# Ruslan361/iterative_solvers

Measured on AMD Instinct MI355X. Metric: cg_iters_per_sec, higher is better.
Workload: dtype f64; 1 GPU; 4096x4096 L-shaped Dirichlet Poisson fp64, matrix-free CG, fixed 2641 iterations; n=4096, unknowns=12574721, rule=rel2

## Files before the change

include/mi355cg.h:

```cpp
#ifndef MI355CG_H
#define MI355CG_H

#include <stddef.h>

#ifdef __cplusplus
extern "C" {
#endif

#define MI355CG_OK            0
#define MI355CG_ERR_INVALID   1
#define MI355CG_ERR_HIP       2
#define MI355CG_ERR_STATE     3

#define MI355CG_F64           0
#define MI355CG_F32_MIXED     1

#define MI355CG_RULE_MSG_MAXNORM  0
#define MI355CG_RULE_REL_2NORM    1

#define MI355CG_STOP_ITERATIONS   0
#define MI355CG_STOP_PRECISION    1
#define MI355CG_STOP_RESIDUAL     2
#define MI355CG_STOP_EXACT_ERROR  3
#define MI355CG_STOP_INTERRUPTED  4
// ... 48 lines not shown
int  mi355cg_set_rhs(mi355cg_handle h, const double *b);
int  mi355cg_setup_on_device(mi355cg_handle h);

int  mi355cg_apply(mi355cg_handle h, const double *x, double *y);
int  mi355cg_apply_device(mi355cg_handle h, const double *x_dev, double *y_dev);

void mi355cg_default_params(mi355cg_params *p, int rule);
int  mi355cg_solve(mi355cg_handle h, const mi355cg_params *params,
                   mi355cg_iter_cb cb, void *user, const volatile int *stop_flag,
                   mi355cg_results *out);
int  mi355cg_get_solution(mi355cg_handle h, double *x);
int  mi355cg_get_recursive_residual(mi355cg_handle h, double *r);
int  mi355cg_get_true_residual(mi355cg_handle h, double *ax_minus_b);

#define MI355CG_PRECOND_NONE    0
#define MI355CG_PRECOND_MG      1
#define MI355CG_PRECOND_MG_ANY  2
int  mi355cg_set_preconditioner(mi355cg_handle h, int kind);
int  mi355cg_apply_preconditioner(mi355cg_handle h, const double *r, double *z);
int  mi355cg_mg_levels(int n, int *levels, int *coarsest_n);
int  mi355cg_mg_hierarchy(int kind, int n, int max_levels, int *levels, int *level_n);

#define MI355CG_CYCLE_F64 0
#define MI355CG_CYCLE_F32 1
int  mi355cg_set_preconditioner_ex(mi355cg_handle h, int kind, int cycle);
int  mi355cg_preconditioner_info(mi355cg_handle h, int *kind, int *cycle, int *levels);

#define MI355CG_SMOOTHER_JACOBI    0
#define MI355CG_SMOOTHER_LINE_X    1
#define MI355CG_SMOOTHER_LINE_Y    2
#define MI355CG_SMOOTHER_LINE_AUTO 3
int  mi355cg_set_smoother(mi355cg_handle h, int smoother);
int  mi355cg_get_smoother(mi355cg_handle h, int *smoother, int *direction);

#define MI355CG_BATCH_MAX 64
int  mi355cg_solve_batch(mi355cg_handle h, const mi355cg_params *params, int nrhs, const double *b, double *x,
                         const volatile int *stop_flag, mi355cg_results *out);
int  mi355cg_solve_batch_device(mi355cg_handle h, const mi355cg_params *params, int nrhs, const double *b_dev, double *x_dev,
                                const volatile int *stop_flag, mi355cg_results *out);
int  mi355cg_batch_release(mi355cg_handle h);

int  mi355cg_set_initial_guess(mi355cg_handle h, const double *x0);
int  mi355cg_set_initial_guess_device(mi355cg_handle h, const double *x0_dev);
int  mi355cg_use_solution_as_initial_guess(mi355cg_handle h);
int  mi355cg_solve_batch_from(mi355cg_handle h, const mi355cg_params *params, int nrhs, const double *b, double *x,
                              const volatile int *stop_flag, mi355cg_results *out);
int  mi355cg_solve_batch_device_from(mi355cg_handle h, const mi355cg_params *params, int nrhs, const double *b_dev, double *x_dev,
                                     const volatile int *stop_flag, mi355cg_results *out);

int  mi355cg_set_shift(mi355cg_handle h, double sigma);
int  mi355cg_get_shift(mi355cg_handle h, double *sigma);
int  mi355cg_time_steps(mi355cg_handle h, const mi355cg_params *params, double tau, double theta, int nsteps,
                        const volatile int *stop_flag, mi355cg_results *out , int *steps_done);
int  mi355cg_get_solution_device(mi355cg_handle h, double *x_dev);

#define MI355CG_EIG_BLOCK_MAX 16
#define MI355CG_EIG_CONVERGED   0
#define MI355CG_EIG_ITERATIONS  1
#define MI355CG_EIG_INTERRUPTED 2
#define MI355CG_EIG_BREAKDOWN   3
typedef struct mi355cg_eig_results {
    int iterations;
    int converged;
    int stop_reason;
    int p_drops;
    double solve_seconds;
} mi355cg_eig_results;
int  mi355cg_eigs(mi355cg_handle h, int nev, int block, double tol, int max_iterations, double *x, double *lambda, double *resid,
                  const volatile int *stop_flag, mi355cg_eig_results *out);
int  mi355cg_eigs_device(mi355cg_handle h, int nev, int block, double tol, int max_iterations, double *x_dev, double *lambda,
                         double *resid, const volatile int *stop_flag, mi355cg_eig_results *out);
int  mi355cg_eigs_release(mi355cg_handle h);
int  mi355cg_block_gram(mi355cg_handle h, int na, const double *a, int nb, const double *b, double *c);
int  mi355cg_block_gram_indexed(mi355cg_handle h, int na, const double *a, int nia, const int *ia, int nb, const double *b,
                                int nib, const int *ib, double *c);
int  mi355cg_block_combine(mi355cg_handle h, int k, const double *s, int m, const double *coef, double *y);
int  mi355cg_rayleigh_ritz(int k, const double *g, const double *hmat, double *theta, double *coef);

int  mi355cg_set_profiling(mi355cg_handle h, int enable);
int  mi355cg_get_kernel_time(mi355cg_handle h, int kernel, double *avg_ms, long long *launches);
int  mi355cg_get_layout(mi355cg_handle h, long long *padded_len, int *pitch_bottom, int *pitch_upper,
                        int *grid_stencil, int *grid_update, int *rows_per_item);
int  mi355cg_get_xfold(mi355cg_handle h, int *depth, int *extra_buffers);

#define MI355CG_SOLVE_LAUNCHES 0
#define MI355CG_SOLVE_ONCHIP   1
int  mi355cg_set_solve_mode(mi355cg_handle h, int mode);
int  mi355cg_get_solve_mode(mi355cg_handle h, int *mode, long long *onchip_launches_last_solve);
int  mi355cg_onchip_plan(int n, int *threads, int *lds_bytes, int *elems_per_thread);

#define MI355CG_MANY_MAX 65536
int  mi355cg_solve_many(mi355cg_handle h, const mi355cg_params *params, int nsys, const double *b, double *x, const double *sigma,
                        const volatile int *stop_flag, mi355cg_results *out);
int  mi355cg_solve_many_from(mi355cg_handle h, const mi355cg_params *params, int nsys, const double *b, double *x, const double *sigma,
                             const volatile int *stop_flag, mi355cg_results *out);
int  mi355cg_solve_many_device(mi355cg_handle h, const mi355cg_params *params, int nsys, const double *b_dev, double *x_dev,
                               const double *sigma_dev, const volatile int *stop_flag, mi355cg_results *out);
int  mi355cg_solve_many_device_from(mi355cg_handle h, const mi355cg_params *params, int nsys, const double *b_dev, double *x_dev,
                                    const double *sigma_dev, const volatile int *stop_flag, mi355cg_results *out);
int  mi355cg_solve_many_info(mi355cg_handle h, int nsys, int *lds_bytes_per_workgroup, int *workgroups_per_cu, long long *workspace_bytes);

int  mi355cg_slab_rows(int n, int world, int rank, int *y_lo, int *y_hi);
int  mi355cg_create_part(int n, int m, double a, double b, double c, double d, int dtype, int device,
                         int y_lo, int y_hi, int x_lo, int x_hi, mi355cg_handle *out);
int  mi355cg_checksum(mi355cg_handle h, int which, double *out2);
int  mi355cg_create_slab(int n, int m, double a, double b, double c, double d, int dtype, int device,
                         int y_lo, int y_hi, mi355cg_handle *out);
int  mi355cg_owned_range(mi355cg_handle h, long long *packed_begin, long long *packed_len, int *y_lo, int *y_hi);
int  mi355cg_dist_begin(mi355cg_handle h, const mi355cg_params *params, void *stream);
int  mi355cg_dist_reduce(mi355cg_handle h, int which , int with_rows, void *stream);
int  mi355cg_dist_sums_ptr(mi355cg_handle h, int which, void **dev_ptr, int *count );
int  mi355cg_dist_record_layout(mi355cg_handle h, int *header, int *row_slot, int *width);
int  mi355cg_dist_scatter_ghosts(mi355cg_handle h, int vector ,
                                 const double *gathered_records, int nranks, int rank, void *stream);
int  mi355cg_dist_stencil(mi355cg_handle h, const double *gathered_update_sums, int nranks, int estride,
                          int rows , void *stream);
int  mi355cg_dist_flip(mi355cg_handle h);
int  mi355cg_dist_update(mi355cg_handle h, const double *gathered_stencil_sums, int nranks, int estride,
                         int rows , void *stream);
int  mi355cg_dist_update_reads_ghosts(mi355cg_handle h);
int  mi355cg_dist_check(mi355cg_handle h, const double *gathered_update_sums, int nranks, int estride, void *stream);
int  mi355cg_dist_summary(mi355cg_handle h, mi355cg_results *out, int *done);
int  mi355cg_dist_finish(mi355cg_handle h, void *stream);
int  mi355cg_dist_history(mi355cg_handle h, int iteration, double *precision, double *residual, double *error);
int  mi355cg_dist_halo(mi355cg_handle h, int vector ,
                       void **send_lo, void **recv_lo, long long *n_send_lo,
                       void **send_hi, void **recv_hi, long long *n_send_hi);
int  mi355cg_dist_halo_recv_counts(mi355cg_handle h, long long *n_from_lo, long long *n_from_hi);

#define MI355CG_DECOMP_ROWS 0
#define MI355CG_DECOMP_2D   1
typedef struct mi355cg_team_s *mi355cg_team;
typedef struct mi355cg_halo_msg {
    int id;
    int peer;
    int send;
    int kind;
    int y0, y1, x0, x1;
    long long count;
} mi355cg_halo_msg;
int  mi355cg_decompose(int n, int world, int decomp, int rank, int *y_lo, int *y_hi, int *x_lo, int *x_hi);
int  mi355cg_halo_plan(int n, int world, int decomp, int rank, int max_msgs, int *n_msgs, mi355cg_halo_msg *msgs);
int  mi355cg_debug_plan(int n, int world, int decomp, int rank, int which, int *n_panels, int *panels,
                        int *grid, int *n_items, int *cls);
int  mi355cg_team_create_local(int n, int m, double a, double b, double c, double d, int world,
                               const int *devices, int ndevices, int decomp, mi355cg_team *out);
int  mi355cg_team_unique_id(void *id128);
int  mi355cg_team_create_rccl(int n, int m, double a, double b, double c, double d, int world, int rank, int device,
                              const void *id128, int decomp, mi355cg_team *out);
void mi355cg_team_destroy(mi355cg_team t);
int  mi355cg_team_solve(mi355cg_team t, const mi355cg_params *params, mi355cg_iter_cb cb, void *user,
                        const volatile int *stop_flag, mi355cg_results *out);
int  mi355cg_team_info(mi355cg_team t, int *world, int *nlocal, int *decomp, long long *size);
int  mi355cg_team_describe(mi355cg_team t, char *buf, int len);
int  mi355cg_team_part(mi355cg_team t, int local_index, mi355cg_handle *part, int *rank);
int  mi355cg_team_get_vector(mi355cg_team t, int which, double *global_packed);
int  mi355cg_team_checksum(mi355cg_team t, int which, double *out2);
int  mi355cg_team_set_vector(mi355cg_team t, int which, const double *global_packed);
int  mi355cg_team_set_dtype(mi355cg_team t, int dtype);
int  mi355cg_team_setup_on_device(mi355cg_team t);
int  mi355cg_team_set_profiling(mi355cg_team t, int enable);
int  mi355cg_team_phase_times(mi355cg_team t, double *kernel_ms, double *comm_ms, double *wall_ms);

#ifdef __cplusplus
}
#endif
// ... 2 lines not shown
```

iterative_solvers_amd/_capi.py:

```python
from __future__ import annotations

import ctypes as C
import os

import numpy as np

from . import build as _build

OK, ERR_INVALID, ERR_HIP, ERR_STATE = 0, 1, 2, 3
F64, F32_MIXED = 0, 1
RULE_MSG_MAXNORM, RULE_REL_2NORM = 0, 1
STOP_ITERATIONS, STOP_PRECISION, STOP_RESIDUAL, STOP_EXACT_ERROR, STOP_INTERRUPTED = range(5)

EXPORTS = [
    "mi355cg_create", "mi355cg_create_csr", "mi355cg_set_true_solution", "mi355cg_destroy", "mi355cg_last_error", "mi355cg_version", "mi355cg_size",
    "mi355cg_get_rhs", "mi355cg_get_true_solution", "mi355cg_get_node_coords", "mi355cg_set_rhs",
    "mi355cg_apply", "mi355cg_apply_device", "mi355cg_default_params", "mi355cg_solve",
    "mi355cg_get_solution", "mi355cg_get_recursive_residual", "mi355cg_get_true_residual",
    "mi355cg_set_profiling", "mi355cg_get_kernel_time", "mi355cg_get_layout",
    "mi355cg_slab_rows", "mi355cg_create_slab", "mi355cg_owned_range", "mi355cg_dist_begin",
    "mi355cg_dist_reduce", "mi355cg_dist_sums_ptr", "mi355cg_dist_record_layout", "mi355cg_dist_scatter_ghosts", "mi355cg_dist_stencil", "mi355cg_dist_flip",
    "mi355cg_dist_update", "mi355cg_dist_update_reads_ghosts", "mi355cg_dist_check", "mi355cg_dist_summary", "mi355cg_dist_finish", "mi355cg_dist_history",
    "mi355cg_dist_halo", "mi355cg_dist_halo_recv_counts",
    "mi355cg_create_part", "mi355cg_checksum", "mi355cg_decompose", "mi355cg_halo_plan",
    "mi355cg_team_create_local", "mi355cg_team_unique_id", "mi355cg_team_create_rccl", "mi355cg_team_destroy",
    "mi355cg_team_solve", "mi355cg_team_info", "mi355cg_team_part", "mi355cg_team_get_vector", "mi355cg_team_set_vector", "mi355cg_team_checksum",
    "mi355cg_team_set_profiling", "mi355cg_team_phase_times", "mi355cg_team_describe", "mi355cg_setup_on_device", "mi355cg_team_setup_on_device", "mi355cg_debug_plan",
    "mi355cg_team_set_dtype", "mi355cg_set_preconditioner", "mi355cg_apply_preconditioner", "mi355cg_mg_levels",
    "mi355cg_mg_hierarchy", "mi355cg_set_preconditioner_ex", "mi355cg_preconditioner_info",
    "mi355cg_solve_batch", "mi355cg_solve_batch_device", "mi355cg_batch_release", "mi355cg_get_xfold",
    "mi355cg_set_initial_guess", "mi355cg_set_initial_guess_device", "mi355cg_use_solution_as_initial_guess",
    "mi355cg_solve_batch_from", "mi355cg_solve_batch_device_from",
    "mi355cg_set_shift", "mi355cg_get_shift", "mi355cg_time_steps", "mi355cg_get_solution_device",
    "mi355cg_eigs", "mi355cg_eigs_device", "mi355cg_eigs_release", "mi355cg_block_gram", "mi355cg_block_gram_indexed",
    "mi355cg_block_combine", "mi355cg_rayleigh_ritz",
    "mi355cg_set_smoother", "mi355cg_get_smoother",
    "mi355cg_set_solve_mode", "mi355cg_get_solve_mode", "mi355cg_onchip_plan",
    "mi355cg_solve_many", "mi355cg_solve_many_from", "mi355cg_solve_many_device", "mi355cg_solve_many_device_from", "mi355cg_solve_many_info",
]
DECOMP_ROWS, DECOMP_2D = 0, 1
PRECOND_NONE, PRECOND_MG, PRECOND_MG_ANY = 0, 1, 2
CYCLE_F64, CYCLE_F32 = 0, 1
SOLVE_LAUNCHES, SOLVE_ONCHIP = 0, 1
SMOOTHER_JACOBI, SMOOTHER_LINE_X, SMOOTHER_LINE_Y, SMOOTHER_LINE_AUTO = 0, 1, 2, 3
BATCH_MAX = 64
MANY_MAX = 65536
EIG_BLOCK_MAX = 16
EIG_BASIS_MAX = 48
EIG_CONVERGED, EIG_ITERATIONS, EIG_INTERRUPTED, EIG_BREAKDOWN = range(4)


class Params(C.Structure):
    _fields_ = [("rule", C.c_int), ("max_iterations", C.c_int),
                ("eps_precision", C.c_double), ("eps_residual", C.c_double),
                ("eps_exact_error", C.c_double), ("eps_rel", C.c_double),
                ("use_true_solution", C.c_int), ("callback_every", C.c_int),
                ("diagnostics", C.c_int), ("sync_every", C.c_int), ("fixed_iterations", C.c_int),
                ("inner_eps", C.c_double)]


class Results(C.Structure):
    _fields_ = [("iterations", C.c_int), ("converged", C.c_int), ("stop_reason", C.c_int),
                ("final_residual_norm", C.c_double), ("final_precision", C.c_double),
                ("final_error_norm", C.c_double), ("r_norm2", C.c_double),
                ("initial_r_norm2", C.c_double), ("solve_seconds", C.c_double),
                ("refine_true_rel", C.c_double), ("refine_outer", C.c_int), ("loop_seconds", C.c_double)]


class EigResults(C.Structure):
    _fields_ = [("iterations", C.c_int), ("converged", C.c_int), ("stop_reason", C.c_int), ("p_drops", C.c_int),
                ("solve_seconds", C.c_double)]


class HaloMsg(C.Structure):
    _fields_ = [("id", C.c_int), ("peer", C.c_int), ("send", C.c_int), ("kind", C.c_int),
                ("y0", C.c_int), ("y1", C.c_int), ("x0", C.c_int), ("x1", C.c_int), ("count", C.c_longlong)]


ITER_CB = C.CFUNCTYPE(None, C.c_void_p, C.c_int, C.c_double, C.c_double, C.c_double)
_DP = np.ctypeslib.ndpointer(dtype=np.float64, flags="C_CONTIGUOUS")

_lib = None


class Mi355cgError(RuntimeError):
    def __init__(self, code: int, text: str):
        super().__init__(f"mi355cg error {code}: {text}")
        self.code = code


def lib_path() -> str:
    return _build.LIB_PATH


def load():
    global _lib
    if _lib is not None:
        return _lib
    path = os.environ.get("MI355CG_LIB") or _build.LIB_PATH
    if path == _build.LIB_PATH and _build.needs_build():
        try:
            _build.build()
        except Exception as e:
            if not os.path.exists(path):
                raise RuntimeError(f"libmi355cg.so is missing and could not be built: {e}") from e
    try:
        import torch
    except ImportError:
        pass
    L = C.CDLL(path)
    H = C.c_void_p
    L.mi355cg_create.argtypes = [C.c_int, C.c_int] + [C.c_double] * 4 + [C.c_int, C.c_int, C.POINTER(H)]
    _IPn = np.ctypeslib.ndpointer(dtype=np.int32, flags="C_CONTIGUOUS")
# ... 18 lines not shown
    L.mi355cg_get_kernel_time.argtypes = [H, C.c_int, C.POINTER(C.c_double), C.POINTER(C.c_longlong)]
    L.mi355cg_get_layout.argtypes = [H, C.POINTER(C.c_longlong)] + [C.POINTER(C.c_int)] * 5
    LLP, IP, VPP = C.POINTER(C.c_longlong), C.POINTER(C.c_int), C.POINTER(C.c_void_p)
    L.mi355cg_slab_rows.argtypes = [C.c_int, C.c_int, C.c_int, IP, IP]
    L.mi355cg_create_slab.argtypes = [C.c_int, C.c_int] + [C.c_double] * 4 + [C.c_int] * 4 + [C.POINTER(H)]
    L.mi355cg_owned_range.argtypes = [H, LLP, LLP, IP, IP]
    L.mi355cg_dist_begin.argtypes = [H, C.POINTER(Params), C.c_void_p]
    L.mi355cg_dist_reduce.argtypes = [H, C.c_int, C.c_int, C.c_void_p]
    L.mi355cg_dist_sums_ptr.argtypes = [H, C.c_int, VPP, IP]
    L.mi355cg_dist_record_layout.argtypes = [H, IP, IP, IP]
    L.mi355cg_dist_scatter_ghosts.argtypes = [H, C.c_int, C.c_void_p, C.c_int, C.c_int, C.c_void_p]
    L.mi355cg_dist_stencil.argtypes = [H, C.c_void_p, C.c_int, C.c_int, C.c_int, C.c_void_p]
    L.mi355cg_dist_flip.argtypes = [H]
    L.mi355cg_dist_update.argtypes = [H, C.c_void_p, C.c_int, C.c_int, C.c_int, C.c_void_p]
    L.mi355cg_dist_update_reads_ghosts.argtypes = [H]
    L.mi355cg_dist_check.argtypes = [H, C.c_void_p, C.c_int, C.c_int, C.c_void_p]
    L.mi355cg_dist_summary.argtypes = [H, C.POINTER(Results), IP]
    L.mi355cg_dist_finish.argtypes = [H, C.c_void_p]
    DBP = C.POINTER(C.c_double)
    L.mi355cg_dist_history.argtypes = [H, C.c_int, DBP, DBP, DBP]
    L.mi355cg_dist_halo.argtypes = [H, C.c_int, VPP, VPP, LLP, VPP, VPP, LLP]
    L.mi355cg_dist_halo_recv_counts.argtypes = [H, LLP, LLP]
    L.mi355cg_create_part.argtypes = [C.c_int, C.c_int] + [C.c_double] * 4 + [C.c_int] * 6 + [C.POINTER(H)]
    L.mi355cg_checksum.argtypes = [H, C.c_int, DBP]
    L.mi355cg_decompose.argtypes = [C.c_int] * 4 + [IP] * 4
    L.mi355cg_halo_plan.argtypes = [C.c_int] * 5 + [IP, C.POINTER(HaloMsg)]
    L.mi355cg_team_create_local.argtypes = [C.c_int, C.c_int] + [C.c_double] * 4 + [C.c_int, IP, C.c_int, C.c_int, C.POINTER(H)]
    L.mi355cg_team_unique_id.argtypes = [C.c_void_p]
    L.mi355cg_team_create_rccl.argtypes = [C.c_int, C.c_int] + [C.c_double] * 4 + [C.c_int, C.c_int, C.c_int, C.c_void_p, C.c_int, C.POINTER(H)]
    L.mi355cg_team_destroy.argtypes = [H]
    L.mi355cg_team_destroy.restype = None
    L.mi355cg_team_solve.argtypes = [H, C.POINTER(Params), ITER_CB, C.c_void_p, C.c_void_p, C.POINTER(Results)]
    L.mi355cg_team_info.argtypes = [H, IP, IP, IP, LLP]
    L.mi355cg_team_part.argtypes = [H, C.c_int, C.POINTER(H), IP]
    L.mi355cg_team_get_vector.argtypes = [H, C.c_int, _DP]
    L.mi355cg_team_set_vector.argtypes = [H, C.c_int, _DP]
    L.mi355cg_team_checksum.argtypes = [H, C.c_int, DBP]
    L.mi355cg_debug_plan.argtypes = [C.c_int] * 5 + [IP, IP, IP, IP, IP]
    L.mi355cg_setup_on_device.argtypes = [H]
    L.mi355cg_team_setup_on_device.argtypes = [H]
    L.mi355cg_team_set_dtype.argtypes = [H, C.c_int]
    L.mi355cg_team_set_profiling.argtypes = [H, C.c_int]
    L.mi355cg_team_phase_times.argtypes = [H, DBP, DBP, DBP]
    L.mi355cg_team_describe.argtypes = [H, C.c_char_p, C.c_int]
    L.mi355cg_set_preconditioner.argtypes = [H, C.c_int]
    L.mi355cg_set_preconditioner_ex.argtypes = [H, C.c_int, C.c_int]
    L.mi355cg_preconditioner_info.argtypes = [H, IP, IP, IP]
    L.mi355cg_apply_preconditioner.argtypes = [H, _DP, _DP]
    L.mi355cg_mg_levels.argtypes = [C.c_int, IP, IP]
    L.mi355cg_mg_hierarchy.argtypes = [C.c_int, C.c_int, C.c_int, IP, IP]
    L.mi355cg_solve_batch.argtypes = [H, C.POINTER(Params), C.c_int, C.c_void_p, C.c_void_p, C.c_void_p, C.POINTER(Results)]
    L.mi355cg_solve_batch_device.argtypes = [H, C.POINTER(Params), C.c_int, C.c_void_p, C.c_void_p, C.c_void_p, C.POINTER(Results)]
    L.mi355cg_batch_release.argtypes = [H]
    L.mi355cg_set_initial_guess.argtypes = [H, C.c_void_p]
    L.mi355cg_set_initial_guess_device.argtypes = [H, C.c_void_p]
    L.mi355cg_use_solution_as_initial_guess.argtypes = [H]
    L.mi355cg_solve_batch_from.argtypes = [H, C.POINTER(Params), C.c_int, C.c_void_p, C.c_void_p, C.c_void_p, C.POINTER(Results)]
    L.mi355cg_solve_batch_device_from.argtypes = [H, C.POINTER(Params), C.c_int, C.c_void_p, C.c_void_p, C.c_void_p, C.POINTER(Results)]
    L.mi355cg_set_shift.argtypes = [H, C.c_double]
    L.mi355cg_get_shift.argtypes = [H, DBP]
    L.mi355cg_time_steps.argtypes = [H, C.POINTER(Params), C.c_double, C.c_double, C.c_int, C.c_void_p, C.POINTER(Results), IP]
    L.mi355cg_get_solution_device.argtypes = [H, C.c_void_p]
    if hasattr(L, "mi355cg_eigs"):
        for fn in (L.mi355cg_eigs, L.mi355cg_eigs_device):
            fn.argtypes = [H, C.c_int, C.c_int, C.c_double, C.c_int, C.c_void_p, C.c_void_p, C.c_void_p, C.c_void_p, C.POINTER(EigResults)]
        L.mi355cg_eigs_release.argtypes = [H]
        L.mi355cg_block_gram.argtypes = [H, C.c_int, C.c_void_p, C.c_int, C.c_void_p, C.c_void_p]
        L.mi355cg_block_gram_indexed.argtypes = [H, C.c_int, C.c_void_p, C.c_int, C.c_void_p, C.c_int, C.c_void_p, C.c_int, C.c_void_p, C.c_void_p]
        L.mi355cg_block_combine.argtypes = [H, C.c_int, C.c_void_p, C.c_int, C.c_void_p, C.c_void_p]
        L.mi355cg_rayleigh_ritz.argtypes = [C.c_int, C.c_void_p, C.c_void_p, C.c_void_p, C.c_void_p]
    if hasattr(L, "mi355cg_set_smoother"):
        L.mi355cg_set_smoother.argtypes = [H, C.c_int]
        L.mi355cg_get_smoother.argtypes = [H, IP, IP]
    if hasattr(L, "mi355cg_set_solve_mode"):
        L.mi355cg_set_solve_mode.argtypes = [H, C.c_int]
        L.mi355cg_get_solve_mode.argtypes = [H, IP, LLP]
        L.mi355cg_onchip_plan.argtypes = [C.c_int, IP, IP, IP]
    if hasattr(L, "mi355cg_solve_many"):
        for fn in (L.mi355cg_solve_many, L.mi355cg_solve_many_from, L.mi355cg_solve_many_device, L.mi355cg_solve_many_device_from):
            fn.argtypes = [H, C.POINTER(Params), C.c_int, C.c_void_p, C.c_void_p, C.c_void_p, C.c_void_p, C.POINTER(Results)]
        L.mi355cg_solve_many_info.argtypes = [H, C.c_int, IP, IP, LLP]
    if hasattr(L, "mi355cg_get_xfold"):
        L.mi355cg_get_xfold.argtypes = [H, IP, IP]
    _lib = L
    return L


def check(rc: int):
    if rc != OK:
        raise Mi355cgError(rc, load().mi355cg_last_error().decode("utf-8", "replace"))
```

iterative_solvers_amd/csrc/cg_kernels.h:

```cpp
#pragma once
#include <hip/hip_runtime.h>
#include <cfloat>
#include <cmath>
#include "solve_loop.h"
#include "item_table.h"

namespace mi355cg {

#ifdef MI355CG_WAVE_TIMING
constexpr int kWtWaves = 16384, kWtStamps = 6;
__device__ unsigned long long g_wave_dbg[2][kWtStamps * kWtWaves];
#define MI355CG_WT_BEGIN unsigned long long wt_[kWtStamps]; for (int i_ = 0; i_ < kWtStamps; ++i_) wt_[i_] = 0; wt_[0] = wall_clock64();
#define MI355CG_WT_STAMP(I) wt_[I] = wall_clock64();
#define MI355CG_WT_MID wt_[kWtStamps - 2] = wall_clock64();
#define MI355CG_WT_END(K) do { if ((threadIdx.x & 63) == 0) { const int w_ = blockIdx.x * 4 + threadIdx.x / 64; \
    if (w_ < kWtWaves) { wt_[kWtStamps - 1] = wall_clock64(); for (int i_ = 0; i_ < kWtStamps; ++i_) g_wave_dbg[K][kWtStamps * w_ + i_] = wt_[i_]; } } } while (0)
#else
#define MI355CG_WT_BEGIN
#define MI355CG_WT_STAMP(I)
#define MI355CG_WT_MID
#define MI355CG_WT_END(K)
#endif

struct StateLite { double alpha, rr, rr_prev, rz, r0norm; int it, done, first, stop; };
// ... 765 lines not shown
    const T alpha = (T)alpha_d;

    dd s_rr = dd_zero(), s_d2 = dd_zero(), s_e2 = dd_zero();
    double s_rmax = 0, s_dmax = 0, s_emax = 0;
    const long long stride = (long long)gridDim.x * kBlock;
    vec_t* __restrict__ X = reinterpret_cast<vec_t*>(a.x);
    vec_t* __restrict__ R = reinterpret_cast<vec_t*>(a.r);
    const vec_t* __restrict__ Pp = reinterpret_cast<const vec_t*>(a.p);
    const vec_t* __restrict__ Q = reinterpret_cast<const vec_t*>(a.ap);
    const vec_t* __restrict__ Uu = reinterpret_cast<const vec_t*>(a.u);

    auto elem = [&](long long i, const vec_t& x0, const vec_t& pv, const vec_t& r0, const vec_t& qv, const vec_t& uv) {
        vec_t xn, rn;
#pragma unroll
        for (int j = 0; j < VEC; ++j) {
            xn[j] = x0[j] + alpha * pv[j];
            rn[j] = r0[j] - alpha * qv[j];
            const double rd = (double)rn[j];
            dd_acc_prod(s_rr, rd, rd);
            s_rmax = fmax(s_rmax, fabs(rd));
            const double dx = (double)(xn[j] - x0[j]);
            s_dmax = fmax(s_dmax, fabs(dx));
            dd_acc_prod(s_d2, dx, dx);
            if (HAS_U) {
                const double ee = (double)(xn[j] - uv[j]);
                s_emax = fmax(s_emax, fabs(ee));
                dd_acc_prod(s_e2, ee, ee);
            }
        }
        X[i] = xn; R[i] = rn;
    };
    long long i = a.begin + (long long)blockIdx.x * kBlock + threadIdx.x;
    const long long end = a.begin + a.nvec;
    for (; i + stride < end; i += 2 * stride) {
        const long long j0 = i, j1 = i + stride;
        const vec_t xa = X[j0], pa = Pp[j0], ra = R[j0], qa = Q[j0];
        const vec_t xb = X[j1], pb = Pp[j1], rb = R[j1], qb = Q[j1];
        vec_t ua{}, ub{}; if (HAS_U) { ua = Uu[j0]; ub = Uu[j1]; }
        elem(j0, xa, pa, ra, qa, ua);
        elem(j1, xb, pb, rb, qb, ub);
    }
    if (i < end) {
        const vec_t x0 = X[i], pv = Pp[i], r0 = R[i], qv = Q[i];
        vec_t uv{}; if (HAS_U) uv = Uu[i];
        elem(i, x0, pv, r0, qv, uv);
    }

    const dd t_rr = block_reduce_dd(s_rr, lds);
    const double t_rmax = block_reduce<true>(s_rmax, lds);
    const double t_dmax = block_reduce<true>(s_dmax, lds);
    const dd t_d2 = block_reduce_dd(s_d2, lds);
    double t_emax = 0; dd t_e2 = dd_zero();
    if (HAS_U) { t_emax = block_reduce<true>(s_emax, lds); t_e2 = block_reduce_dd(s_e2, lds); }
    if (threadIdx.x == 0) {
        const int b = blockIdx.x, st = a.strideB;
        a.partB[FB_RR * st + b] = t_rr.hi; a.partB[(FB_RR + FB_LO) * st + b] = t_rr.lo;
        a.partB[FB_D2 * st + b] = t_d2.hi; a.partB[(FB_D2 + FB_LO) * st + b] = t_d2.lo;
        a.partB[FB_E2 * st + b] = t_e2.hi; a.partB[(FB_E2 + FB_LO) * st + b] = t_e2.lo;
        a.partB[FB_RMAX * st + b] = t_rmax; a.partB[FB_DMAX * st + b] = t_dmax; a.partB[FB_EMAX * st + b] = t_emax;
        if (blockIdx.x == 0) {
            CgState* o = a.s_out;
            if (a.init == 1) {
                *o = CgState{};
                o->first = 1;
            } else {
                copy_state(a.s_out, a.s_in);
                if (a.init == 2) {
                    if (s.done) o->rr = s.rr_prev;
                    o->done = 0; o->reason = 0; o->converged = 0; o->alpha = 0.0; o->r0norm = a.r0norm_resume;
                    for (int i = 0; i < kRing; ++i) o->alpha_hist[i] = 0.0;
                } else { o->it = s.it + 1; o->first = 0; o->alpha = alpha_d; o->rz = rz; o->alpha_hist[(s.it + 1) & (kRing - 1)] = alpha_d; }
            }
        }
    }
}

template <typename T>
struct FreshArgs {
    long long begin, nvec;
    const T* b; T* x; T* r; T* p0; const T* u;
    double* partB; int strideB;
    CgState* s_out;
};
template <typename T, int VEC, bool HAS_U>
__global__ __launch_bounds__(kBlock) void k_init_fresh(const FreshArgs<T> a) {
    typedef typename VecOf<T, VEC>::type vec_t;
    __shared__ double lds[2 * kWaves];
    dd s_rr = dd_zero(), s_e2 = dd_zero();
    double s_rmax = 0, s_emax = 0;
    const long long stride = (long long)gridDim.x * kBlock;
    const vec_t* __restrict__ B = reinterpret_cast<const vec_t*>(a.b);
    const vec_t* __restrict__ Uu = reinterpret_cast<const vec_t*>(a.u);
    vec_t* __restrict__ X = reinterpret_cast<vec_t*>(a.x);
    vec_t* __restrict__ R = reinterpret_cast<vec_t*>(a.r);
    vec_t* __restrict__ P = reinterpret_cast<vec_t*>(a.p0);
    vec_t zero;
#pragma unroll
    for (int j = 0; j < VEC; ++j) zero[j] = (T)0;
    const long long end = a.begin + a.nvec;
    for (long long i = a.begin + (long long)blockIdx.x * kBlock + threadIdx.x; i < end; i += stride) {
        const vec_t bv = B[i];
        vec_t uv; if (HAS_U) uv = Uu[i];
#pragma unroll
        for (int j = 0; j < VEC; ++j) {
            const double rd = (double)bv[j];
            dd_acc_prod(s_rr, rd, rd);
            s_rmax = fmax(s_rmax, fabs(rd));
            if (HAS_U) {
                const double ee = (double)((T)0 - uv[j]);
                s_emax = fmax(s_emax, fabs(ee));
                dd_acc_prod(s_e2, ee, ee);
            }
        }
        X[i] = zero; R[i] = bv; P[i] = zero;
    }
    const dd t_rr = block_reduce_dd(s_rr, lds);
    const double t_rmax = block_reduce<true>(s_rmax, lds);
    double t_emax = 0; dd t_e2 = dd_zero();
    if (HAS_U) { t_emax = block_reduce<true>(s_emax, lds); t_e2 = block_reduce_dd(s_e2, lds); }
    if (threadIdx.x == 0) {
        const int b = blockIdx.x, st = a.strideB;
        a.partB[FB_RR * st + b] = t_rr.hi; a.partB[(FB_RR + FB_LO) * st + b] = t_rr.lo;
        a.partB[FB_D2 * st + b] = 0.0; a.partB[(FB_D2 + FB_LO) * st + b] = 0.0;
        a.partB[FB_E2 * st + b] = t_e2.hi; a.partB[(FB_E2 + FB_LO) * st + b] = t_e2.lo;
        a.partB[FB_RMAX * st + b] = t_rmax; a.partB[FB_DMAX * st + b] = 0.0; a.partB[FB_EMAX * st + b] = t_emax;
        if (blockIdx.x == 0) { *a.s_out = CgState{}; a.s_out->first = 1; }
    }
}

template <typename T>
struct GuessArgs {
    long long begin, nvec;
    const T* b; const T* ax; const T* x; T* r; T* p0; const T* u;
    double* partB; int strideB;
    double* partG; int strideG;
    CgState* s_out;
};
template <typename T, int VEC, bool HAS_U>
__global__ __launch_bounds__(kBlock) void k_init_guess(const GuessArgs<T> a) {
    typedef typename VecOf<T, VEC>::type vec_t;
    __shared__ double lds[2 * kWaves];
    dd s_rr = dd_zero(), s_bb = dd_zero(), s_e2 = dd_zero();
    double s_rmax = 0, s_emax = 0;
    const long long stride = (long long)gridDim.x * kBlock;
    const vec_t* __restrict__ B = reinterpret_cast<const vec_t*>(a.b);
    const vec_t* __restrict__ AX = reinterpret_cast<const vec_t*>(a.ax);
    const vec_t* __restrict__ X = reinterpret_cast<const vec_t*>(a.x);
    const vec_t* __restrict__ Uu = reinterpret_cast<const vec_t*>(a.u);
    vec_t* __restrict__ R = reinterpret_cast<vec_t*>(a.r);
    vec_t* __restrict__ P = reinterpret_cast<vec_t*>(a.p0);
    vec_t zero;
#pragma unroll
    for (int j = 0; j < VEC; ++j) zero[j] = (T)0;
    const long long end = a.begin + a.nvec;
    for (long long i = a.begin + (long long)blockIdx.x * kBlock + threadIdx.x; i < end; i += stride) {
        const vec_t bv = B[i], av = AX[i];
        vec_t xv, uv; if (HAS_U) { xv = X[i]; uv = Uu[i]; }
        vec_t rv;
#pragma unroll
        for (int j = 0; j < VEC; ++j) {
            rv[j] = bv[j] - av[j];
            const double rd = (double)rv[j], bd = (double)bv[j];
            dd_acc_prod(s_rr, rd, rd);
            dd_acc_prod(s_bb, bd, bd);
            s_rmax = fmax(s_rmax, fabs(rd));
            if (HAS_U) {
                const double ee = (double)(xv[j] - uv[j]);
                s_emax = fmax(s_emax, fabs(ee));
                dd_acc_prod(s_e2, ee, ee);
            }
        }
        R[i] = rv; P[i] = zero;
    }
    const dd t_rr = block_reduce_dd(s_rr, lds);
    const double t_rmax = block_reduce<true>(s_rmax, lds);
    double t_emax = 0; dd t_e2 = dd_zero();
    if (HAS_U) { t_emax = block_reduce<true>(s_emax, lds); t_e2 = block_reduce_dd(s_e2, lds); }
    const dd t_bb = block_reduce_dd(s_bb, lds);
    if (threadIdx.x == 0) {
        const int b = blockIdx.x, st = a.strideB;
        a.partB[FB_RR * st + b] = t_rr.hi; a.partB[(FB_RR + FB_LO) * st + b] = t_rr.lo;
        a.partB[FB_D2 * st + b] = 0.0; a.partB[(FB_D2 + FB_LO) * st + b] = 0.0;
        a.partB[FB_E2 * st + b] = t_e2.hi; a.partB[(FB_E2 + FB_LO) * st + b] = t_e2.lo;
        a.partB[FB_RMAX * st + b] = t_rmax; a.partB[FB_DMAX * st + b] = 0.0; a.partB[FB_EMAX * st + b] = t_emax;
        a.partG[b] = t_bb.hi; a.partG[a.strideG + b] = t_bb.lo;
        if (blockIdx.x == 0) { *a.s_out = CgState{}; a.s_out->first = 1; }
    }
}
__global__ __launch_bounds__(kBlock) void k_guess_state(const double* partB, int strideB, const double* partG, int strideG, int n,
                                                        CgState* s, double* norms) {
    __shared__ double lds[2 * kWaves];
    const double rr = dd_value(reduce_parts_dd(partB + FB_RR * strideB, partB + (FB_RR + FB_LO) * strideB, n, 1, lds));
    const double bb = dd_value(reduce_parts_dd(partG, partG + strideG, n, 1, lds));
    if (threadIdx.x == 0) { s->r0norm = sqrt(bb); s->first = 2; norms[0] = sqrt(rr); norms[1] = sqrt(bb); }
}

template <typename T>
struct UpdateStArgs {
    Geom g;
    ItemTab tab;
    const T* p;
    const T* pprev[kRing - 1];
    T* r; T* x; const T* u;
    const double* partA; int nA, strideA, esA;
    RecSrc src;
    double* partB; int strideB, slotB;
    const CgState* s_in; CgState* s_out;
    int rule;
    int reverse;
    const int* stop_req;
    FlagSpec fl;
    QueueSpec dq;
    double* fold_alpha;
    int fold_mask;
};

template <typename T, int VEC, int XM, bool HAS_U, int DEPTH, bool DESC, bool TEAM, bool QUEUE>
__global__ __launch_bounds__(kBlock) void k_update_st(const UpdateStArgs<T> a) {
    static_assert(DEPTH >= 1 && DEPTH <= 3, "see k_stencil");
    typedef typename VecOf<T, VEC>::type vec_t;
    __shared__ double lds[2 * kWaves];
    const Geom& g = a.g;
    const int lane = threadIdx.x & (kWave - 1);
    const int wave = __builtin_amdgcn_readfirstlane(threadIdx.x / kWave);
    MI355CG_WT_BEGIN
    const StartRec rec = start_rec(a.reverse ? a.tab.start_rev : a.tab.start, wave);
    const ItemSeq seq = rec.seq;
    constexpr bool FULL = XM == 1;
    constexpr int NP = XM >= 2 ? XM - 1 : 0;
    struct Raw { vec_t p, r, x, u, pp[NP > 0 ? NP : 1]; T pe; };

    StateLite s{};
    PreParts pre_lean{0.0, 0.0, 0.0, 0.0}, pre_rz_lean{0.0, 0.0, 0.0, 0.0};
    if (!TEAM) {
        s = load_state_lite(a.s_in);
        const rsrc_t rs_part = make_rsrc(a.partA);
        const int fa = a.strideA * (int)sizeof(double);
        pre_lean = prefetch_parts_buf(rs_part, FA_PAP * fa, FA_LO * fa, a.nA, a.esA);
        if (FULL) pre_rz_lean = prefetch_parts_buf(rs_part, FA_RZ * fa, FA_LO * fa, a.nA, a.esA);
    }

    int f_item = seq.first;
    bool f_have = f_item < seq.end;
    ItemAddr F{};
    int f_idx = 0, f_so = 0, f_y = 0;
    rsrc_t rs_p = make_rsrc(a.p), rs_r = rs_p, rs_x = rs_p, rs_u = rs_p;
    rsrc_t rs_pp[NP > 0 ? NP : 1] = {rs_p};
    const int dq_nsub = min(kQueueSubs, (int)(gridDim.x / kXcds)), dq_sub = (int)(blockIdx.x / kXcds) % dq_nsub;
    int* const dq = (QUEUE && a.dq.mine) ? a.dq.mine + ((int)(blockIdx.x % kXcds) * kQueueSubs + dq_sub) * kQueuePitch : nullptr;
    if (QUEUE && a.dq.other && blockIdx.x == 0 && threadIdx.x < kXcds * kQueueSubs) a.dq.other[threadIdx.x * kQueuePitch] = 0;
    int dq_ticket = 0;
    auto enter = [&](const ItemUni& u) {
        if (QUEUE && dq) dq_ticket = queue_take(dq, lane);
        F = item_addr<T, VEC, DESC>(g, u, lane);
        rs_p = make_rsrc(a.p + F.base_el);
        rs_r = make_rsrc(a.r + F.base_el);
        rs_x = make_rsrc(XM != 0 ? a.x + F.base_el : a.p + F.base_el);
#pragma unroll
        for (int i = 0; i < NP; ++i) rs_pp[i] = make_rsrc(a.pprev[i] + F.base_el);
        rs_u = make_rsrc((FULL && HAS_U) ? a.u + F.base_el : a.p + F.base_el);
        f_idx = -1; f_so = F.so_first; f_y = DESC ? F.ystart + 1 : F.ystart - 1;
    };
    auto fetch = [&](bool may_switch = true) -> Raw {
        if (may_switch && f_have && f_idx > F.nrows) {
            f_item = (QUEUE && dq) ? seq.begin + seq.step + __builtin_amdgcn_readfirstlane(dq_ticket) * dq_nsub + dq_sub : f_item + seq.step;
            f_have = f_item < seq.end;
            if (f_have) enter(item_uniform<DESC>(g, decode_item(a.tab, a.reverse ? seq.end - 1 - (f_item - seq.begin) : f_item), (int)sizeof(T)));
        }
        const bool own = f_have && f_idx >= 0 && f_idx < F.nrows;
        int vo = own ? F.vo_own : (f_idx < 0 ? F.vo_first : F.vo_last);
        if (!f_have) vo = kOob;
        const int vown = own ? F.vo_own : kOob;
        Raw w;
        w.p = buf_load<vec_t>(rs_p, vo, f_so);
        w.r = buf_load<vec_t>(rs_r, vown, f_so);
        if (XM != 0) w.x = buf_load<vec_t>(rs_x, vown, f_so);
#pragma unroll
        for (int i = 0; i < NP; ++i) w.pp[i] = buf_load<vec_t>(rs_pp[i], vown, f_so);
        if (FULL && HAS_U) w.u = buf_load<vec_t>(rs_u, vown, f_so);
        w.pe = buf_load<T>(rs_p, own ? F.ve_own : kOob, f_so);
        if (DESC) { f_so -= row_step<T>(g, f_y - 1); --f_y; } else { f_so += row_step<T>(g, f_y); ++f_y; }
        ++f_idx;
        return w;
    };

    bool c_have = f_have;
    ItemAddr C{};
    int c_idx = -1, c_so = 0, c_y = 0;
    bool in_j[VEC];
#pragma unroll
    for (int j = 0; j < VEC; ++j) in_j[j] = false;
    rsrc_t rs_ro = rs_p, rs_xo = rs_p;
    auto promote = [&]() {
        C = F;
        rs_ro = make_rsrc(a.r + C.base_el);
        rs_xo = make_rsrc(XM != 0 ? a.x + C.base_el : a.p + C.base_el);
        c_idx = -1; c_so = C.so_c0; c_y = C.ystart;
        const int xint0 = C.bot ? g.half + 1 : 1;
#pragma unroll
        for (int j = 0; j < VEC; ++j) in_j[j] = (C.x + j >= xint0) && (C.x + j <= g.N - 1);
    };

    if (f_have) { enter(rec.u); promote(); }
    Raw q[DEPTH];
#pragma unroll
    for (int k = 0; k < DEPTH; ++k) q[k] = fetch(false);
    MI355CG_WT_STAMP(3)
    int stop_word = 0;
    if (blockIdx.x == 0 && a.stop_req) stop_word = scalar_load(a.stop_req);

    double alpha_d, rz = 0.0;
    if (!TEAM) {
        if (s.done) { if (blockIdx.x == 0 && threadIdx.x == 0) copy_state(a.s_out, a.s_in); return; }
        MI355CG_WT_STAMP(1)
        const double pap = dd_value(reduce_parts_dd_pre(pre_lean, a.partA + FA_PAP * a.strideA, a.partA + (FA_PAP + FA_LO) * a.strideA, a.nA, a.esA, lds));
        if (a.rule == 0) {
            rz = FULL ? dd_value(reduce_parts_dd_pre(pre_rz_lean, a.partA + FA_RZ * a.strideA, a.partA + (FA_RZ + FA_LO) * a.strideA, a.nA, a.esA, lds))
                      : dd_value(reduce_parts_dd(a.partA + FA_RZ * a.strideA, a.partA + (FA_RZ + FA_LO) * a.strideA, a.nA, a.esA, lds));
            alpha_d = rz / pap;
        } else {
            alpha_d = s.rr / pap;
        }
        MI355CG_WT_STAMP(2)
    } else if (a.src.mbox) {
        __shared__ double recs[kMaxRecDst * kRecWords];
        const PreParts pre = prefetch_parts(a.partA + FA_PAP * a.strideA, a.partA + (FA_PAP + FA_LO) * a.strideA, a.nA, 1);
        PreParts pre_rz{0, 0, 0, 0};
        if (FULL) pre_rz = prefetch_parts(a.partA + FA_RZ * a.strideA, a.partA + (FA_RZ + FA_LO) * a.strideA, a.nA, 1);
        s = load_state_lite(a.s_in);
        if (s.done) {
            if (threadIdx.x == 0) { store_flagged_zero(a.fl, a.slotB + blockIdx.x, FB_LL_COUNT); if (blockIdx.x == 0) copy_state(a.s_out, a.s_in); }
            return;
        }
        {
            double* R = recs + a.src.me * kRecWords;
            if (threadIdx.x < kRecWords) R[threadIdx.x] = 0.0;
            const dd pap = reduce_parts_dd_pre(pre, a.partA + FA_PAP * a.strideA, a.partA + (FA_PAP + FA_LO) * a.strideA, a.nA, 1, lds);
            dd rzd = dd_zero();
            if (a.rule == 0) rzd = FULL ? reduce_parts_dd_pre(pre_rz, a.partA + FA_RZ * a.strideA, a.partA + (FA_RZ + FA_LO) * a.strideA, a.nA, 1, lds)
// ... 101 lines not shown

    MI355CG_WT_END(1);
    const dd t_rr = block_reduce_dd(s_rr, lds);
    const double t_rmax = block_reduce<true>(s_rmax, lds);
    double t_dmax = 0, t_emax = 0; dd t_d2 = dd_zero(), t_e2 = dd_zero();
    if (FULL) { t_dmax = block_reduce<true>(s_dmax, lds); t_d2 = block_reduce_dd(s_d2, lds); }
    if (FULL && HAS_U) { t_emax = block_reduce<true>(s_emax, lds); t_e2 = block_reduce_dd(s_e2, lds); }
    if (threadIdx.x == 0) {
        const int b = a.slotB + blockIdx.x, st = a.strideB;
        a.partB[FB_RR * st + b] = t_rr.hi; a.partB[(FB_RR + FB_LO) * st + b] = t_rr.lo;
        a.partB[FB_D2 * st + b] = t_d2.hi; a.partB[(FB_D2 + FB_LO) * st + b] = t_d2.lo;
        a.partB[FB_E2 * st + b] = t_e2.hi; a.partB[(FB_E2 + FB_LO) * st + b] = t_e2.lo;
        a.partB[FB_RMAX * st + b] = t_rmax; a.partB[FB_DMAX * st + b] = t_dmax; a.partB[FB_EMAX * st + b] = t_emax;
        if (TEAM && a.fl.part) {
            const double v[FB_LL_COUNT] = {t_rr.hi, t_d2.hi, t_e2.hi, t_rr.lo, t_d2.lo, t_e2.lo, t_rmax, t_dmax, t_emax, (blockIdx.x == 0 && stop_word) ? 1.0 : 0.0};
            store_flagged(a.fl, b, FB_LL_COUNT, v);
        }
        if (blockIdx.x == 0) {
            copy_state(a.s_out, a.s_in);
            CgState* o = a.s_out;
            o->it = s.it + 1; o->first = 0; o->alpha = alpha_d; o->rz = rz; o->alpha_hist[(s.it + 1) & (kRing - 1)] = alpha_d;
            o->stop = stop_word != 0;
            if (a.fold_alpha) a.fold_alpha[(s.it + 1) & a.fold_mask] = alpha_d;
        }
    }
}

struct CheckArgs {
    const double* partB; int nB, strideB, esB;
    RecSrc src;
    const CgState* s_in;
    CgState* summary;
    HistEntry* hist;
    RuleParams rp;
    int want_diag;
};
__global__ __launch_bounds__(kBlock) void k_check(const CheckArgs a) {
    __shared__ double lds[2 * kWaves];
    const StateLite s = load_state_lite(a.s_in);
    if (s.done) { if (threadIdx.x == 0) copy_state(a.summary, a.s_in); return; }
    Decision d;
    if (a.src.mbox) {
        __shared__ double recs[kMaxRecDst * kRecWords];
        own_record_B(recs, a.src.me, a.partB, a.nB, a.strideB, 2, lds);
        if (!gather_records(a.src, recs)) { if (threadIdx.x == 0) fail_transport(a.summary, a.s_in); return; }
        d = decide_from_records(s, a.rp, recs, a.src.world, true, true);
    } else d = reduce_and_decide(s, a.rp, a.partB, a.nB, a.strideB, a.esB, 1, lds);
    if (threadIdx.x == 0) write_state_after_decision(a.summary, a.hist, a.s_in, s, d);
}

template <typename T> struct FlushArgs { const T* p[kRing - 1]; T a[kRing - 1]; int n; };
template <typename T, int VEC>
__global__ __launch_bounds__(kBlock) void k_flush_x(const Geom g, const ItemTab tab, T* x, const FlushArgs<T> f) {
    typedef typename VecOf<T, VEC>::type vec_t;
    const int lane = threadIdx.x & (kWave - 1);
    const int wave = __builtin_amdgcn_readfirstlane(threadIdx.x / kWave);
    for (int item = blockIdx.x * kWaves + wave; item < tab.nitems; item += gridDim.x * kWaves) {
        const Item it = decode_item(tab, item);
        const int x0 = it.strip * (kWave * VEC) + lane * VEC;
        if (x0 < (it.ya <= g.half ? g.cb : 0) || x0 >= g.xlim) continue;
        for (int y = it.ya; y <= it.yb; ++y) {
            const long long off = row_off(g, y) - g.base0 + x0;
            vec_t xn = *reinterpret_cast<const vec_t*>(x + off);
#pragma unroll
            for (int k = 0; k < kRing - 1; ++k) if (k < f.n) {
                const vec_t pv = *reinterpret_cast<const vec_t*>(f.p[k] + off);
#pragma unroll
                for (int j = 0; j < VEC; ++j) xn[j] = xn[j] + f.a[k] * pv[j];
            }
            *reinterpret_cast<vec_t*>(x + off) = xn;
        }
    }
}

constexpr int kFoldMax = 32;
struct FoldTable { const double* p[kFoldMax]; double alpha[kFoldMax]; };
struct FoldArgs {
    long long begin, nvec;
    double* x;
    const FoldTable* tab;
    const CgState* s;
    int mask;
    int flush_it;
};
template <int NS, bool NT>
__device__ inline void fold_block(VecOf<double, 2>::type& xv, const FoldTable* tab, int k0, int mask, long long i) {
    typedef VecOf<double, 2>::type vec_t;
    const vec_t* P[NS]; double al[NS]; vec_t v[NS];
#pragma unroll
    for (int j = 0; j < NS; ++j) {
        const int slot = (k0 + j) & mask;
        P[j] = reinterpret_cast<const vec_t*>(scalar_load(&tab->p[slot]));
        al[j] = scalar_load(&tab->alpha[slot]);
    }
#pragma unroll
    for (int j = 0; j < NS; ++j) v[j] = NT ? __builtin_nontemporal_load(P[j] + i) : P[j][i];
#pragma unroll
    for (int j = 0; j < NS; ++j) { xv[0] = xv[0] + al[j] * v[j][0]; xv[1] = xv[1] + al[j] * v[j][1]; }
}
template <bool NT>
__global__ __launch_bounds__(kBlock) void k_fold_x(const FoldArgs a) {
    typedef VecOf<double, 2>::type vec_t;
    const int it = a.flush_it >= 0 ? a.flush_it : scalar_load(&a.s->it);
    int n = it & a.mask;
    if (a.flush_it < 0) {
        if (scalar_load(&a.s->done) || n != 0 || it == 0) return;
        n = a.mask + 1;
    }
    if (n == 0) return;
    vec_t* __restrict__ X = reinterpret_cast<vec_t*>(a.x);
    const long long stride = (long long)gridDim.x * kBlock, end = a.begin + a.nvec;
    for (long long i = a.begin + (long long)blockIdx.x * kBlock + threadIdx.x; i < end; i += stride) {
        vec_t xv = X[i];
        int k = it - n + 1;
        for (; k + 8 <= it + 1; k += 8) fold_block<8, NT>(xv, a.tab, k, a.mask, i);
        if (k + 4 <= it + 1) { fold_block<4, NT>(xv, a.tab, k, a.mask, i); k += 4; }
        if (k + 2 <= it + 1) { fold_block<2, NT>(xv, a.tab, k, a.mask, i); k += 2; }
        if (k <= it) fold_block<1, NT>(xv, a.tab, k, a.mask, i);
        X[i] = xv;
    }
}

template <typename T, int VEC>
__global__ __launch_bounds__(kBlock) void k_checksum(const Geom g, const ItemTab tab, const T* v, double* part) {
    typedef typename VecOf<T, VEC>::type vec_t;
    __shared__ double lds[2 * kWaves];
    const int lane = threadIdx.x & (kWave - 1);
    const int wave = __builtin_amdgcn_readfirstlane(threadIdx.x / kWave);
    dd s1 = dd_zero(), s2 = dd_zero();
    for (int item = blockIdx.x * kWaves + wave; item < tab.nitems; item += gridDim.x * kWaves) {
        const Item it = decode_item(tab, item);
        const int x0 = it.strip * (kWave * VEC) + lane * VEC;
        if (x0 < (it.ya <= g.half ? g.cb : 0) || x0 >= g.xlim) continue;
        for (int y = it.ya; y <= it.yb; ++y) {
            const vec_t t = *reinterpret_cast<const vec_t*>(v + (row_off(g, y) - g.base0 + x0));
#pragma unroll
            for (int j = 0; j < VEC; ++j) { s1 = dd_add(s1, dd{(double)t[j], 0.0}); dd_acc_prod(s2, (double)t[j], (double)t[j]); }
        }
    }
    const dd t1 = block_reduce_dd(s1, lds), t2 = block_reduce_dd(s2, lds);
    if (threadIdx.x == 0) {
        const int n = gridDim.x, b = blockIdx.x;
        part[b] = t1.hi; part[n + b] = t1.lo; part[2 * n + b] = t2.hi; part[3 * n + b] = t2.lo;
    }
}

template <typename T>
__global__ __launch_bounds__(kBlock) void k_err_maxnorm(long long begin, long long len, const T* x, const T* u, double* part) {
    __shared__ double lds[2 * kWaves];
    const long long stride = (long long)gridDim.x * kBlock;
    double m = 0.0;
    for (long long i = begin + (long long)blockIdx.x * kBlock + threadIdx.x; i < begin + len; i += stride)
        m = fmax(m, fabs((double)(x[i] - u[i])));
    const double t = block_reduce<true>(m, lds);
    if (threadIdx.x == 0) part[blockIdx.x] = t;
}

__global__ __launch_bounds__(kBlock) void k_residual_to_f32(long long total, long long own_begin, long long own_len,
                                                           const double* b, const double* ax, float* rf, double* part) {
    __shared__ double lds[2 * kWaves];
    const long long stride = (long long)gridDim.x * kBlock;
    double s = 0.0;
    for (long long i = (long long)blockIdx.x * kBlock + threadIdx.x; i < total; i += stride) {
        const double d = b[i] - ax[i];
        rf[i] = (float)d;
        if (i >= own_begin && i < own_begin + own_len) s += d * d;
    }
    const double t = block_reduce<false>(s, lds);
    if (threadIdx.x == 0) part[blockIdx.x] = t;
}
__global__ __launch_bounds__(kBlock) void k_accumulate_f32(long long begin, long long len, double* x, const float* d) {
    const long long stride = (long long)gridDim.x * kBlock;
    for (long long i = begin + (long long)blockIdx.x * kBlock + threadIdx.x; i < begin + len; i += stride) x[i] += (double)d[i];
}

struct RecordArgs {
    const double* part; int n, stride;
    int nsum, lo_off;
    int max_first, nmax;
    double* rec; int header, row_slot;
    const double* v; long long off_lo, off_hi; int len_lo, len_hi;
};
__global__ __launch_bounds__(kBlock) void k_make_record(const RecordArgs a) {
    __shared__ double lds[2 * kWaves];
    if (blockIdx.x == 0) {
        for (int f = 0; f < a.nsum; ++f) {
            const dd t = reduce_parts_dd(a.part + f * a.stride, a.part + (f + a.lo_off) * a.stride, a.n, 1, lds);
            if (threadIdx.x == 0) { a.rec[f] = t.hi; a.rec[f + a.lo_off] = t.lo; }
        }
        for (int f = a.max_first; f < a.max_first + a.nmax; ++f) {
            const double t = reduce_parts<true>(a.part + f * a.stride, a.n, 1, lds);
            if (threadIdx.x == 0) a.rec[f] = t;
        }
        return;
    }
    if (!a.v) return;
// ... 90 lines not shown
```

iterative_solvers_amd/csrc/mi355cg.hip:

```cpp
#include "../../include/mi355cg.h"
#include "cg_kernels.h"
#include "device_buffer.h"
#include "csr_kernels.h"
#include "grid_setup.h"
#include "mg_kernels.h"
#include "mg_batch_kernels.h"
#include "eig_kernels.h"
#include "mg_line_kernels.h"
#include "mg_kernels_f32.h"
#include "step_kernels.h"
#include "onchip_kernels.h"

#include <algorithm>
#include <cfloat>
#include <chrono>
#include <cstdarg>
#include <cstddef>
#include <cstdint>
#include <cstdio>
#include <cstdlib>
#include <cstring>
#include <memory>
#include <string>
#include <thread>
// ... 110 lines not shown
    Buf<double> mat_h;
    Buf<double> red;
    Buf<double> stage;
};

struct OnchipManyWs {
    int cap = 0;
    Buf<double> vec;
    Buf<double> small;
    Buf<CgState> s, summary;
    Buf<int> done;
    Buf<CgState> summary_h;
    Buf<double> small_h;
    Buf<int> done_h;
    Buf<double> stage;
    long long stage_cap = 0;
};

}

struct mi355cg_ctx {
    int device = 0;
    int dtype = MI355CG_F64;
    hipStream_t stream = nullptr;
    GridParams gp;
    Geom g{};
    int s_lo = 0, s_hi = 0;
    long long storage_len = 0;
    long long pk_begin = 0, pk_len = 0;
    PackGeom pg{};
    Plan whole, interior, edge;
    Plan whole32;
    Buf<ItemDesc> plan_items[4];
    Buf<StartRec> plan_start[4][2];
    int depth = 2;
    bool has_gc = false;
    int nB_own = 0;
    int strideA = 0, strideB = 0;

    Buf<double> x, r, p[kRing], ap, b, u;
    int xsteps = 4;
    Buf<double> scratch[2];
    Buf<float> xf, rf, pf[kRing], apf;
    Buf<double> packed;
    Buf<double> partA, partB, partR;
    Buf<double> sumsA, sumsB;
    int rec_width = 0;
    mi355cg_params dist_prm{};
    bool dist_active = false, is_slab = false;
    Buf<CgState> sA, sB, summary;
    Buf<int> qctr;
    int dyn_rows = 0;
    Buf<int> stop_h;
    int* stop_dev = nullptr;
    Buf<HistEntry> hist;
    Buf<CgState> summary_h;
    Buf<HistEntry> hist_h;
    Buf<double> partR_h;

    std::vector<double> rhs_h, u_h;
    bool host_rhs_valid = true, host_u_valid = true;
    bool have_u_dev = false, solved = false;
    bool guess_pending = false;
    bool x_is_guess = false;
    Buf<double> guess_part;
    Buf<double> guess_norms_h;
    double sigma = 0.0;
    int smoother = MI355CG_SMOOTHER_JACOBI;
    Buf<double> step_b;
    bool is_csr = false;
    long long csr_n = 0, csr_nnz = 0;
    Buf<int> csr_row_map, csr_entries; Buf<double> csr_values;
    int grid_csr = 0, grid_update = 0;
    int cur = 0;
    int nA_dist = 0;
    int xfold = 0;
    double* fold_p[kFoldMax] = {};
    Buf<double> fold_own[kFoldMax];
    int fold_extra = 0;
    Buf<FoldTable> fold_tab;
    int fcur = 0;
    int fold_grid = 0;
    bool fold_nt = true;

    struct ChunkGraph { int m, cur; std::vector<char> flags; hipGraphExec_t exec; };
    std::vector<ChunkGraph> graphs;
    mi355cg_params graph_prm{};
    bool graph_stop = false;
    int use_graph = -1;
    int solve_mode = MI355CG_SOLVE_LAUNCHES;
    long long onchip_launches = 0;

    hipEvent_t ev_loop[2] = {nullptr, nullptr};
    std::unique_ptr<MgHier> mg;
    std::unique_ptr<MgBatchWs> batch;
    std::unique_ptr<EigWs> eig;
    std::unique_ptr<OnchipManyWs> many;
    bool profiling = false;
    EventPool events;
    std::vector<std::pair<hipEvent_t, hipEvent_t>> ev_pairs[2];
    double kernel_ms[2] = {0, 0};
    long long kernel_launches[2] = {0, 0};
};

namespace {

long long phys_start(const Geom& g, int y) { return row_off(g, y) + (y <= g.half ? g.cb : 0); }
long long phys_end(const Geom& g, int y) { return phys_start(g, y) + (y <= g.half ? g.Pb : g.Pu); }
int strips_total(const GridParams& gp, int vec) { return (gp.n - 1) / (kWave * vec) + 1; }
int first_bottom_strip(const GridParams& gp, int vec) { return (gp.half + 1) / (kWave * vec); }

void own_cols(const mi355cg_ctx* c, int y, int* xa, int* xb) {
    const int lo = y <= c->gp.half ? c->gp.half + 1 : 1, hi = c->gp.n;
    *xa = std::max(lo, c->s_lo * kStripCols);
    *xb = std::max(*xa, std::min(hi, c->s_hi * kStripCols));
}

void build_geom(mi355cg_ctx* c, int vec, int y_lo, int y_hi) {
    Geom& g = c->g;
    const GridParams& gp = c->gp;
    g.N = gp.n; g.half = gp.half;
    g.Pu = (int)round_up(g.N + 1, 32);
    g.cb = g.half & ~31;
    g.Pb = g.Pu - g.cb;
    g.xlim = (int)round_up(g.N + 1, vec);
    g.y_lo = y_lo; g.y_hi = y_hi;
    g.base0 = 0;
    g.base0 = phys_start(g, y_lo - 1);
    c->storage_len = phys_end(g, y_hi + 1) - g.base0;
    g.own_begin = phys_start(g, y_lo) - g.base0;
    g.own_len = phys_end(g, y_hi) - phys_start(g, y_lo);
    g.A = gp.A; g.xk = gp.x_k; g.yk = gp.y_k;
    PackGeom& pg = c->pg;
    pg.g = g;
    const int yb0 = y_lo, yb1 = std::min(y_hi, gp.half), yu0 = std::max(y_lo, gp.half + 1), yu1 = y_hi;
    int xa = 0, xb = 0;
    pg.nb_rows = std::max(0, yb1 - yb0 + 1); pg.yb0 = yb0;
    own_cols(c, gp.half, &xa, &xb); pg.xb0 = xa; pg.wb = pg.nb_rows ? xb - xa : 0;
    pg.nu_rows = std::max(0, yu1 - yu0 + 1); pg.yu0 = yu0;
    own_cols(c, gp.half + 1, &xa, &xb); pg.xu0 = xa; pg.wu = pg.nu_rows ? xb - xa : 0;
    pg.pk_len = (long long)pg.nb_rows * pg.wb + (long long)pg.nu_rows * pg.wu;
    c->pk_len = pg.pk_len;
    c->pk_begin = packed_row_begin(gp, y_lo);
}

int region_rects(const GridParams& gp, int vec, int ya, int yb, int sa, int sb, Rect out[2]) {
    const int ns_all = strips_total(gp, vec), s0b = first_bottom_strip(gp, vec);
    int nr = 0;
    sb = std::min(sb, ns_all);
    if (ya <= gp.half && yb >= 1) {
        const int s0 = std::max(sa, s0b);
        if (s0 < sb) out[nr++] = Rect{std::max(ya, 1), std::min(yb, gp.half), s0, sb, (sa > s0b ? 1 : 0) | (sb < ns_all ? 2 : 0)};
    }
    if (yb > gp.half && sa < sb)
        out[nr++] = Rect{std::max(ya, gp.half + 1), std::min(yb, gp.n - 1), sa, sb, (sa > 0 ? 1 : 0) | (sb < ns_all ? 2 : 0)};
    return nr;
}

PlanKnobs env_knobs() {
    PlanKnobs kn;
    kn.target_waves = env_int("MI355CG_WAVES", 2048); kn.max_blocks = env_int("MI355CG_BLOCKS", 512);
    { const char* v = getenv("MI355CG_ITEM_ROWS"); kn.item_rows = (v && *v) ? std::max(1, atoi(v)) : 0; }
    kn.xcd_classes = env_int("MI355CG_XCD_CLASSES", 1);
    return kn;
}
Plan make_plan(const std::vector<Rect>& rects, int max_rows, int fixed_ty = 0, int dyn_rows = 0) { return make_plan(rects, env_knobs(), max_rows, fixed_ty, dyn_rows); }
// ... 46 lines not shown
    c->use_graph = env_int("MI355CG_GRAPH", -1);
    c->nB_own = c->whole.grid;
}

template <typename T>
int upload(const std::vector<T>& src, Buf<T>& dst, const char* what = nullptr) {
    Buf<T> fresh;
    if (int rc = Buf<T>::device(fresh, (long long)src.size(), what)) return rc;
    if (hipMemcpy(fresh, src.data(), sizeof(T) * src.size(), hipMemcpyHostToDevice) != hipSuccess) {
        const hipError_t e = hipGetLastError();
        return what ? fail(MI355CG_ERR_HIP, "%s", what) : fail(MI355CG_ERR_HIP, "upload of %zu bytes failed: %s", sizeof(T) * src.size(), hipGetErrorString(e));
    }
    dst = std::move(fresh);
    return MI355CG_OK;
}

int upload_item_tables(mi355cg_ctx* c) {
    int k = 0;
    for (Plan* pl : {&c->whole, &c->interior, &c->edge, &c->whole32}) {
        const int slot = k++;
        if (pl->wl.nitems == 0 || pl->grid == 0) continue;
        if (int rc = upload(build_item_table(pl->wl), c->plan_items[slot])) return rc;
        pl->d_items = c->plan_items[slot];
        pl->elem = pl == &c->whole32 ? (int)sizeof(float) : (int)sizeof(double);
        for (int rev = 0; rev < 2; ++rev) {
            if (int rc = upload(build_start_table(pl->wl, pl->grid, c->g, pl->elem, rev != 0), c->plan_start[slot][rev])) return rc;
            pl->d_start[rev] = c->plan_start[slot][rev];
        }
    }
    return MI355CG_OK;
}
ItemTab item_tab(const Plan& pl) { return ItemTab{pl.d_items, pl.d_start[0], pl.d_start[1], pl.wl.nitems}; }

int flat_grid(long long n) { return (int)std::max<long long>(1, std::min<long long>(2048, (n + kBlock - 1) / kBlock)); }

struct PartSrc { const double* ptr; int n, fstride, estride; RecSrc rec; };
struct Where { hipStream_t stream; const Plan* plan; int slot; };

Where whole_part(const mi355cg_ctx* c) { return Where{c->stream, &c->whole, 0}; }
PartSrc own_partB(const mi355cg_ctx* c) { return PartSrc{c->partB, c->nB_own, c->strideB, 1}; }
PartSrc own_partA(const mi355cg_ctx* c) { return PartSrc{c->partA, c->whole.grid, c->strideA, 1}; }

template <typename T, int VEC> Geom kernel_geom(const mi355cg_ctx* c) { Geom g = c->g; g.xlim = (int)round_up(c->g.N + 1, VEC); return g; }

template <typename T, int VEC>
void launch_apply(const mi355cg_ctx* c, const T* v, T* out, const Where& w) {
    if (w.plan->wl.nitems == 0) return;
    StencilArgs<T> a{};
    a.g = kernel_geom<T, VEC>(c); a.tab = item_tab(*w.plan);
    a.pin = v; a.ap = out; a.partA = nullptr;
    hipLaunchKernelGGL((k_stencil<T, VEC, false, false, 2, false, false, false, false>), dim3(w.plan->grid), dim3(kBlock), 0, w.stream, a);
}

struct IterCfg { RuleParams rp; int want_diag; bool has_u; bool x2 = false; bool fold = false; };

template <typename T, int VEC>
void launch_iteration_stencil(mi355cg_ctx* c, const IterCfg& cfg, const T* r, const Buf<T> p[kRing], const Where& w, const PartSrc& pb, const FlagSpec* fl = nullptr) {
    if (w.plan->wl.nitems == 0) return;
    StencilArgs<T> a{};
    a.g = kernel_geom<T, VEC>(c); a.tab = item_tab(*w.plan);
    a.r = r; a.pin = p[c->cur]; a.pout = p[(c->cur + 1) % c->xsteps]; a.ap = nullptr;
    a.partB = pb.ptr; a.nB = pb.n; a.strideB = pb.fstride; a.esB = pb.estride; a.src = pb.rec;
    a.partA = c->partA; a.strideA = c->strideA; a.slotA = w.slot;
    a.s_in = c->sB; a.s_out = c->sA; a.hist = c->hist; a.rp = cfg.rp; a.want_diag = cfg.want_diag;
    a.store_ghosts = c->is_slab ? 1 : 0;
    if (fl) a.fl = *fl;
    if (VEC == 2 && c->dyn_rows > 0 && w.plan == &c->whole) a.dq = QueueSpec{c->qctr, c->qctr + kXcds * kQueueSubs * kQueuePitch};
    const dim3 grid(w.plan->grid), block(kBlock);
    const bool msg = cfg.rp.rule == MI355CG_RULE_MSG_MAXNORM, gc = c->has_gc, d3 = c->depth == 3;
    const bool team = pb.rec.mbox != nullptr || (fl && fl->part), queue = a.dq.mine != nullptr;
#define MI355CG_ST(MSG, D, GC) do { if (team) hipLaunchKernelGGL((k_stencil<T, VEC, true, MSG, D, true, GC, true, VEC == 2>), grid, block, 0, w.stream, a); \
                                    else if (VEC == 2 && queue) hipLaunchKernelGGL((k_stencil<T, VEC, true, MSG, D, true, GC, false, VEC == 2>), grid, block, 0, w.stream, a); \
                                    else hipLaunchKernelGGL((k_stencil<T, VEC, true, MSG, D, true, GC, false, false>), grid, block, 0, w.stream, a); } while (0)
    if constexpr (VEC == 2) {
        if (msg) { if (gc) { if (d3) MI355CG_ST(true, 3, true); else MI355CG_ST(true, 2, true); } else { if (d3) MI355CG_ST(true, 3, false); else MI355CG_ST(true, 2, false); } }
        else     { if (gc) { if (d3) MI355CG_ST(false, 3, true); else MI355CG_ST(false, 2, true); } else { if (d3) MI355CG_ST(false, 3, false); else MI355CG_ST(false, 2, false); } }
    } else {
        if (d3) MI355CG_ST(false, 3, false); else MI355CG_ST(false, 2, false);
    }
#undef MI355CG_ST
}

template <typename T, int VEC>
void launch_iteration_update(mi355cg_ctx* c, const IterCfg& cfg, T* x, T* r, const Buf<T> p[kRing], const T* u, const Where& w, const PartSrc& pa, const FlagSpec* fl = nullptr) {
    if (w.plan->wl.nitems == 0) return;
    UpdateStArgs<T> a{};
    a.g = kernel_geom<T, VEC>(c); a.tab = item_tab(*w.plan);
    a.p = p[c->cur]; a.r = r; a.x = x; a.u = u;
    for (int i = 0; i < kRing - 1; ++i) a.pprev[i] = p[(c->cur + 2 * kRing * c->xsteps - 1 - i) % c->xsteps];
    a.partA = pa.ptr; a.nA = pa.n; a.strideA = pa.fstride; a.esA = pa.estride; a.src = pa.rec;
    a.partB = c->partB; a.strideB = c->strideB; a.slotB = w.slot;
    a.s_in = c->sA; a.s_out = c->sB; a.rule = cfg.rp.rule; a.reverse = 1;
    if (fl) a.fl = *fl;
    if (VEC == 2 && c->dyn_rows > 0 && w.plan == &c->whole) a.dq = QueueSpec{c->qctr + kXcds * kQueueSubs * kQueuePitch, c->qctr};
    if (cfg.fold) { a.fold_alpha = reinterpret_cast<double*>(reinterpret_cast<char*>(c->fold_tab.get()) + offsetof(FoldTable, alpha)); a.fold_mask = c->xfold - 1; }
    a.stop_req = w.slot == 0 ? c->stop_dev : nullptr;
    const dim3 grid(w.plan->grid), block(kBlock);
    const bool d3 = c->depth == 3 && !(cfg.x2 && c->cur == 0 && c->xsteps == 8);
    const bool team = pa.rec.mbox != nullptr || (fl && fl->part), queue = a.dq.mine != nullptr;
#define MI355CG_UST_D(XM, HASU, D) do { if (team) hipLaunchKernelGGL((k_update_st<T, VEC, XM, HASU, D, true, true, VEC == 2>), grid, block, 0, w.stream, a); \
                                        else if (VEC == 2 && queue) hipLaunchKernelGGL((k_update_st<T, VEC, XM, HASU, D, true, false, VEC == 2>), grid, block, 0, w.stream, a); \
                                        else hipLaunchKernelGGL((k_update_st<T, VEC, XM, HASU, D, true, false, false>), grid, block, 0, w.stream, a); } while (0)
#define MI355CG_UST(XM, HASU) do { if (d3) MI355CG_UST_D(XM, HASU, 3); else MI355CG_UST_D(XM, HASU, 2); } while (0)
    if (cfg.x2) {
        if (c->cur != 0 || cfg.fold) MI355CG_UST(0, false); else if (c->xsteps == 8) MI355CG_UST(8, false); else if (c->xsteps == 4) MI355CG_UST(4, false); else MI355CG_UST(2, false);
    }
    else if constexpr (VEC == 2) { if (cfg.has_u) MI355CG_UST(1, true); else MI355CG_UST(1, false); }
#undef MI355CG_UST
#undef MI355CG_UST_D
}

template <typename T, int VEC>
void launch_update_flat(mi355cg_ctx* c, const IterCfg& cfg, T* x, T* r, const T* p, const T* ap, const T* u, hipStream_t stream,
                        int grid, double resume_r0norm = -1.0) {
    UpdateArgs<T> a{};
    a.begin = c->g.own_begin / VEC; a.nvec = c->g.own_len / VEC;
    a.x = x; a.r = r; a.p = p; a.ap = ap; a.u = u;
    a.partA = c->partA; a.nA = 0; a.strideA = c->strideA; a.esA = 1;
    a.partB = c->partB; a.strideB = c->strideB;
    a.s_in = c->sA; a.s_out = c->sB; a.rule = cfg.rp.rule; a.init = 1;
    if (resume_r0norm >= 0.0) { a.init = 2; a.r0norm_resume = resume_r0norm; a.s_in = c->sB; }
    if (cfg.has_u) hipLaunchKernelGGL((k_update<T, VEC, true>), dim3(grid), dim3(kBlock), 0, stream, a);
    else hipLaunchKernelGGL((k_update<T, VEC, false>), dim3(grid), dim3(kBlock), 0, stream, a);
}

template <typename T, int VEC>
void launch_flush_x(const mi355cg_ctx* c, const Plan& plan, T* x, const Buf<T> p[kRing], const CgState& fin, hipStream_t stream) {
    const int pending = fin.it % c->xsteps;
    if (plan.wl.nitems == 0 || pending == 0) return;
    FlushArgs<T> f{};
    f.n = pending;
    for (int j = 0; j < pending; ++j) { const int k = fin.it - pending + 1 + j; f.p[j] = p[k % c->xsteps]; f.a[j] = (T)fin.alpha_hist[k & (kRing - 1)]; }
    hipLaunchKernelGGL((k_flush_x<T, VEC>), dim3(std::max(1, std::min(1024, (plan.wl.nitems + kWaves - 1) / kWaves))), dim3(kBlock), 0, stream,
                       kernel_geom<T, VEC>(c), item_tab(plan), x, f);
}

void launch_fold_x(const mi355cg_ctx* c, int flush_it, hipStream_t stream) {
    FoldArgs a{};
    a.begin = c->g.own_begin / 2; a.nvec = c->g.own_len / 2;
    a.x = c->x; a.tab = c->fold_tab; a.s = c->sB; a.mask = c->xfold - 1; a.flush_it = flush_it;
    const long long one_shot = (a.nvec + kBlock - 1) / kBlock;
    const int grid = (int)std::max<long long>(1, c->fold_grid > 0 ? std::min<long long>(c->fold_grid, one_shot) : one_shot);
    if (c->fold_nt) hipLaunchKernelGGL((k_fold_x<true>), dim3(grid), dim3(kBlock), 0, stream, a);
    else hipLaunchKernelGGL((k_fold_x<false>), dim3(grid), dim3(kBlock), 0, stream, a);
}
void free_fold_ring(mi355cg_ctx* c) {
    for (int k = c->xsteps; k < kFoldMax; ++k) { c->fold_own[k].reset(); c->fold_p[k] = nullptr; }
    c->fold_tab.reset();
    c->fold_extra = 0;
}
bool ensure_fold_ring(mi355cg_ctx* c) {
    if (c->xfold == 0) return false;
    if (c->fold_tab) return true;
    const size_t bytes = sizeof(double) * (size_t)c->storage_len;
    bool ok = true;
    for (int k = 0; k < c->xfold && ok; ++k) {
        if (k < c->xsteps) { c->fold_p[k] = c->p[k]; continue; }
        ok = Buf<double>::device(c->fold_own[k], c->storage_len) == MI355CG_OK && hipMemsetAsync(c->fold_own[k], 0, bytes, c->stream) == hipSuccess;
        c->fold_p[k] = c->fold_own[k];
    }
    FoldTable t{};
    for (int k = 0; k < c->xfold; ++k) t.p[k] = c->fold_p[k];
    ok = ok && Buf<FoldTable>::device(c->fold_tab, 1) == MI355CG_OK &&
         hipMemcpyAsync(c->fold_tab, &t, sizeof t, hipMemcpyHostToDevice, c->stream) == hipSuccess && hipStreamSynchronize(c->stream) == hipSuccess;
    if (!ok) {
        (void)hipGetLastError();
        hipStreamSynchronize(c->stream);
        free_fold_ring(c);
        c->xfold = 0;
        return false;
    }
    c->fold_extra = c->xfold - c->xsteps;
    return true;
}

void launch_check(mi355cg_ctx* c, const IterCfg& cfg, hipStream_t stream, const PartSrc& pb) {
    CheckArgs a{};
    a.partB = pb.ptr; a.nB = pb.n; a.strideB = pb.fstride; a.esB = pb.estride; a.src = pb.rec;
    a.s_in = c->sB; a.summary = c->summary; a.hist = c->hist; a.rp = cfg.rp; a.want_diag = cfg.want_diag;
    hipLaunchKernelGGL(k_check, dim3(1), dim3(kBlock), 0, stream, a);
}

IterCfg make_cfg(const mi355cg_params* prm) {
    IterCfg cfg{};
    const bool msg = prm->rule == MI355CG_RULE_MSG_MAXNORM;
    cfg.rp.rule = prm->rule; cfg.rp.max_iterations = prm->max_iterations;
    cfg.rp.eps_precision = prm->eps_precision; cfg.rp.eps_residual = prm->eps_residual;
    cfg.rp.eps_exact_error = prm->eps_exact_error; cfg.rp.eps_rel = prm->eps_rel;
    cfg.rp.fixed_iterations = prm->fixed_iterations;
    const bool diag = !msg && prm->diagnostics;
    cfg.has_u = (msg && prm->use_true_solution) || diag;
    cfg.rp.use_u = cfg.has_u ? 1 : 0;
    cfg.want_diag = diag ? 1 : 0;
    cfg.x2 = !msg && !diag;
    return cfg;
}

template <typename T>
int upload_packed(mi355cg_ctx* c, const double* host_packed, T* storage) {
    if (c->is_csr) {
        HIPCK(hipMemcpyAsync(storage, host_packed, sizeof(double) * c->pk_len, hipMemcpyHostToDevice, c->stream));
        HIPCK(hipStreamSynchronize(c->stream));
        return MI355CG_OK;
    }
    if (c->is_slab) HIPCK(hipDeviceSynchronize());
    if (c->pk_len == 0) return MI355CG_OK;
    HIPCK(hipMemcpyAsync(c->packed, host_packed, sizeof(double) * c->pk_len, hipMemcpyHostToDevice, c->stream));
    hipLaunchKernelGGL((k_unpack<T>), dim3(flat_grid(c->pk_len)), dim3(kBlock), 0, c->stream, c->pg, c->packed, storage);
    HIPCK(hipGetLastError());
    HIPCK(hipStreamSynchronize(c->stream));
    return MI355CG_OK;
}
template <typename T>
int download_packed(mi355cg_ctx* c, const T* storage, double* host_packed) {
    if (c->is_csr) {
        HIPCK(hipMemcpyAsync(host_packed, storage, sizeof(double) * c->pk_len, hipMemcpyDeviceToHost, c->stream));
        HIPCK(hipStreamSynchronize(c->stream));
        return MI355CG_OK;
    }
    if (c->is_slab) HIPCK(hipDeviceSynchronize());
    if (c->pk_len == 0) return MI355CG_OK;
    hipLaunchKernelGGL((k_pack<T>), dim3(flat_grid(c->pk_len)), dim3(kBlock), 0, c->stream, c->pg, storage, c->packed);
    HIPCK(hipGetLastError());
    HIPCK(hipMemcpyAsync(host_packed, c->packed, sizeof(double) * c->pk_len, hipMemcpyDeviceToHost, c->stream));
    HIPCK(hipStreamSynchronize(c->stream));
    return MI355CG_OK;
}

int ensure_host_copies(mi355cg_ctx* c) {
    if (!c->host_rhs_valid) { c->rhs_h.resize(c->pk_len); if (int rc = download_packed<double>(c, c->b, c->rhs_h.data())) return rc; c->host_rhs_valid = true; }
    if (!c->host_u_valid) { c->u_h.resize(c->pk_len); if (int rc = download_packed<double>(c, c->u, c->u_h.data())) return rc; c->host_u_valid = true; }
    return MI355CG_OK;
}
int ensure_f32_vectors(mi355cg_ctx* c) {
    if (c->xsteps > 4) return fail(MI355CG_ERR_INVALID, "MI355CG_XSTEPS=8 is fp64 only");
    if (c->whole32.wl.nitems == 0) return fail(MI355CG_ERR_INVALID, "the fp32 kernels march 256-column strips: a part of a 2-D decomposition (cut on 128 columns) cannot run them; use row slabs");
    if (c->g.own_begin % 4 != 0 || c->g.own_len % 4 != 0) return fail(MI355CG_ERR_STATE, "a part's owned range is not a whole number of float4");
    Buf<float>* fv[] = {&c->xf, &c->apf, &c->pf[0], &c->pf[1], &c->pf[2], &c->pf[3]};
    for (int k = 0; k < 2 + c->xsteps; ++k)
        if (!*fv[k]) if (int rc = Buf<float>::device_zeroed(*fv[k], c->storage_len, "fp32 vector allocation failed")) return rc;
    HIPCK(hipDeviceSynchronize());
    return MI355CG_OK;
}

int ensure_u_on_device(mi355cg_ctx* c) {
    if (c->have_u_dev) return MI355CG_OK;
    if (!c->host_u_valid) return fail(MI355CG_ERR_STATE, "no exact solution on host or device");
    if (int rc = upload_packed<double>(c, c->u_h.data(), c->u)) return rc;
    c->have_u_dev = true;
    return MI355CG_OK;
}
int ensure_scratch(mi355cg_ctx* c) {
    for (auto& s : c->scratch) if (!s) { if (int rc = Buf<double>::device_zeroed(s, c->storage_len)) return rc; }
    HIPCK(hipDeviceSynchronize());
    return MI355CG_OK;
}

int ensure_guess_ws(mi355cg_ctx* c) {
    if (!c->guess_part) if (int rc = Buf<double>::device(c->guess_part, 2 * (long long)c->strideB + 2)) return rc;
    if (!c->guess_norms_h) if (int rc = Buf<double>::pinned(c->guess_norms_h, 2)) return rc;
    return MI355CG_OK;
}

void clear_graphs(mi355cg_ctx* c) {
    for (auto& g : c->graphs) hipGraphExecDestroy(g.exec);
    c->graphs.clear();
}

void prof_begin(mi355cg_ctx* c, hipEvent_t* e0) {
    if (!c->profiling) return;
    *e0 = c->events.get();
    if (*e0) hipEventRecord(*e0, c->stream);
}
void prof_end(mi355cg_ctx* c, int k, hipEvent_t e0) {
    if (!c->profiling || !e0) return;
    hipEvent_t e1 = c->events.get();
    if (!e1) return;
    hipEventRecord(e1, c->stream);
    c->ev_pairs[k].push_back({e0, e1});
}
void prof_collect(mi355cg_ctx* c) {
    for (int k = 0; k < 2; ++k) {
        double tot = 0; long long n = 0;
        for (auto& pr : c->ev_pairs[k]) {
            float ms = 0;
            if (hipEventElapsedTime(&ms, pr.first, pr.second) == hipSuccess) { tot += ms; ++n; }
        }
        c->kernel_ms[k] = n ? tot / n : 0.0;
        c->kernel_launches[k] = n;
        c->ev_pairs[k].clear();
    }
    c->events.reset();
}

int fetch_state(mi355cg_ctx* c, hipStream_t st) {
    HIPCK(hipMemcpyAsync(c->summary_h, c->summary, sizeof(CgState), hipMemcpyDeviceToHost, st));
    HIPCK(hipMemcpyAsync(c->hist_h, c->hist, sizeof(HistEntry) * kHist, hipMemcpyDeviceToHost, st));
    return MI355CG_OK;
}
int wait_stream_forwarding_stop(mi355cg_ctx* c, const volatile int* stop_flag) {
    if (!stop_flag) { HIPCK(hipStreamSynchronize(c->stream)); return MI355CG_OK; }
    for (;;) {
        if (*stop_flag) *c->stop_h = 1;
        const hipError_t q = hipStreamQuery(c->stream);
        if (q == hipSuccess) break;
        if (q != hipErrorNotReady) HIPCK(q);
        std::this_thread::yield();
    }
    return MI355CG_OK;
}
int loop_timer_begin(mi355cg_ctx* c, hipStream_t st) {
    if (!c->ev_loop[0]) { HIPCK(hipEventCreate(&c->ev_loop[0])); HIPCK(hipEventCreate(&c->ev_loop[1])); }
    HIPCK(hipEventRecord(c->ev_loop[0], st));
    return MI355CG_OK;
}
int loop_timer_end(mi355cg_ctx* c, hipStream_t st) { HIPCK(hipEventRecord(c->ev_loop[1], st)); return MI355CG_OK; }
double loop_timer_seconds(const mi355cg_ctx* c) {
    float ms = 0;
    return hipEventElapsedTime(&ms, c->ev_loop[0], c->ev_loop[1]) == hipSuccess ? 1e-3 * ms : 0.0;
}

}

namespace {

CsrView csr_view(const mi355cg_ctx* c) { return CsrView{c->csr_n, c->csr_row_map, c->csr_entries, c->csr_values}; }

void launch_csr_spmv(mi355cg_ctx* c, const double* x, double* y, const double* r, const CgState* s_in, double* partA) {
    SpmvArgs a{};
    a.A = csr_view(c); a.x = x; a.y = y; a.r = r; a.s_in = s_in; a.partA = partA; a.strideA = c->strideA;
    hipLaunchKernelGGL(k_csr_spmv, dim3(c->grid_csr), dim3(kBlock), 0, c->stream, a);
}

int solve_csr(mi355cg_ctx* c, const mi355cg_params* prm, mi355cg_iter_cb cb, void* user,
              const volatile int* stop_flag, mi355cg_results* out) {
    if (prm->diagnostics) return fail(MI355CG_ERR_INVALID, "per-iteration diagnostics are not available on CSR handles");
    const bool msg = prm->rule == MI355CG_RULE_MSG_MAXNORM;
    IterCfg cfg = make_cfg(prm);
    if (cfg.has_u && !c->have_u_dev) { cfg.has_u = false; cfg.rp.use_u = 0; }
    const auto t0 = std::chrono::steady_clock::now();
    const size_t bytes = sizeof(double) * c->storage_len;
    HIPCK(hipMemsetAsync(c->x, 0, bytes, c->stream));
    HIPCK(hipMemsetAsync(c->p[0], 0, bytes, c->stream));
    HIPCK(hipMemsetAsync(c->ap, 0, bytes, c->stream));
    HIPCK(hipMemcpyAsync(c->r, c->b, bytes, hipMemcpyDeviceToDevice, c->stream));
    c->cur = 0;
    const PartSrc pA{c->partA, c->grid_csr, c->strideA, 1};
    auto update = [&](bool init, bool with_u) {
        UpdateArgs<double> a{};
        a.begin = 0; a.nvec = c->csr_n;
        a.x = c->x; a.r = c->r; a.p = c->p[0]; a.ap = c->ap; a.u = c->u;
        a.partA = pA.ptr; a.nA = pA.n; a.strideA = pA.fstride; a.esA = 1;
        a.partB = c->partB; a.strideB = c->strideB;
        a.s_in = c->sA; a.s_out = c->sB; a.rule = cfg.rp.rule; a.init = init ? 1 : 0;
        if (with_u) hipLaunchKernelGGL((k_update<double, 1, true>), dim3(c->grid_update), dim3(kBlock), 0, c->stream, a);
        else hipLaunchKernelGGL((k_update<double, 1, false>), dim3(c->grid_update), dim3(kBlock), 0, c->stream, a);
    };
    update(true, cfg.has_u);
    HIPCK(hipGetLastError());
    auto poll = [&]() -> int {
        launch_check(c, cfg, c->stream, own_partB(c));
        if (int rc = fetch_state(c, c->stream)) return rc;
        HIPCK(hipStreamSynchronize(c->stream));
        return MI355CG_OK;
    };
    if (int rc = poll()) return rc;
    const double initial_rnorm2 = c->summary_h->rnorm2;
    if (msg && cb) cb(user, 0, DBL_MAX, c->summary_h->rmax, cfg.has_u ? c->summary_h->emax : DBL_MAX);
    const int sync_every = default_sync_every(prm, msg);
    int it_done = 0;
    bool first_chunk = (cb != nullptr || stop_flag != nullptr);
    bool interrupted = false;
    while (!c->summary_h->done) {
        if (stop_flag && *stop_flag) { interrupted = true; break; }
        const int m = chunk_len(prm, msg, sync_every, it_done, first_chunk);
        first_chunk = false;
        for (int k = 0; k < m; ++k) {
            XpayArgs xa{};
            xa.n = c->csr_n; xa.r = c->r; xa.p = c->p[0];
            xa.partB = c->partB; xa.nB = c->grid_update; xa.strideB = c->strideB; xa.esB = 1;
// ... 1060 lines not shown
    }
    hipLaunchKernelGGL(k_mgb_unpack, dim3(flat_grid(c->pk_len), n), dim3(kBlock), 0, c->stream, c->pg, vlen, (const double*)T.packed, T.vec);
    HIPCK(hipGetLastError());
    return MI355CG_OK;
}

}

extern "C" {

const char* mi355cg_last_error(void) { return g_err.c_str(); }
const char* mi355cg_version(void) { return "mi355cg 0.2 (gfx950)"; }

static const char* onchip_refusal(const mi355cg_ctx* c) {
    static char buf[160];
    if (c->is_csr) return "the on-chip solve keeps the grid's direction in LDS: a CSR handle has no grid";
    if (c->is_slab) return "the on-chip solve is one workgroup on one GPU: this handle owns one part of a decomposed grid";
    if (c->dtype != MI355CG_F64) return "the on-chip solve is fp64 only: this handle was created with MI355CG_F32_MIXED";
    if (c->mg) return "the on-chip solve runs plain CG: this handle has a preconditioner (mi355cg_set_preconditioner(h, MI355CG_PRECOND_NONE) first)";
    if (!onchip_supported(c->gp.n)) {
        snprintf(buf, sizeof buf, "the on-chip solve takes grids up to N = %d (the direction must fit in one CU's LDS): this handle has N = %d", kOnchipMaxN, c->gp.n);
        return buf;
    }
    return nullptr;
}
static int create_state(mi355cg_ctx* c, const char* what) {
    if (int rc = Buf<double>::device_zeroed(c->partA, (long long)FA_COUNT * c->strideA)) return rc;
    if (int rc = Buf<double>::device_zeroed(c->partB, (long long)FB_COUNT * c->strideB)) return rc;
    if (int rc = Buf<double>::device_zeroed(c->partR, 2048)) return rc;
    for (Buf<CgState>* s : {&c->sA, &c->sB, &c->summary}) if (int rc = Buf<CgState>::device_zeroed(*s, 1, what)) return rc;
    if (int rc = Buf<HistEntry>::device_zeroed(c->hist, kHist, what)) return rc;
    if (int rc = Buf<CgState>::pinned(c->summary_h, 1, what)) return rc;
    if (int rc = Buf<HistEntry>::pinned(c->hist_h, kHist, what)) return rc;
    return Buf<double>::pinned(c->partR_h, 2048, what);
}

static int create_impl(int n, int m, double a, double b, double c_, double d, int dtype, int device,
                       int y_lo, int y_hi, int s_lo, int s_hi, bool part, mi355cg_handle* out) {
    if (!out) return fail(MI355CG_ERR_INVALID, "out is null");
    *out = nullptr;
    if (dtype != MI355CG_F64 && dtype != MI355CG_F32_MIXED) return fail(MI355CG_ERR_INVALID, "unknown dtype %d", dtype);
    GridParams gp;
    if (!grid_params_init(&gp, n, m, a, b, c_, d))
        return fail(MI355CG_ERR_INVALID, "grid %dx%d rejected: the L-shaped index map is only consistent for n == m, even, >= 6", n, m);
    int ndev = 0;
    if (hipGetDeviceCount(&ndev) != hipSuccess || ndev <= 0)
        return fail(MI355CG_ERR_HIP, "no HIP device available (libmi355cg has no CPU fallback)");
    if (device < 0 || device >= ndev) return fail(MI355CG_ERR_INVALID, "device %d out of range (0..%d)", device, ndev - 1);
    HIPCK(hipSetDevice(device));

    const int ns_all = strips_total(gp, 2);
    if (!part) { y_lo = 1; y_hi = gp.n - 1; s_lo = 0; s_hi = ns_all; }
    if (y_lo < 1 || y_hi > gp.n - 1 || y_lo > y_hi)
        return fail(MI355CG_ERR_INVALID, "part rows [%d, %d] outside 1..%d", y_lo, y_hi, gp.n - 1);
    if (s_lo < 0 || s_hi > ns_all || s_lo >= s_hi)
        return fail(MI355CG_ERR_INVALID, "part strips [%d, %d) outside 0..%d", s_lo, s_hi, ns_all);
    if (dtype == MI355CG_F32_MIXED && part) return fail(MI355CG_ERR_INVALID, "F32_MIXED is single-GPU only");
    mi355cg_ctx* c = new mi355cg_ctx();
    c->device = device; c->dtype = dtype; c->gp = gp; c->is_slab = part;
    c->s_lo = s_lo; c->s_hi = s_hi;
    build_geom(c, 2, y_lo, y_hi);
    build_plans(c);
    c->strideA = std::max({c->whole.grid, c->interior.grid + c->edge.grid, c->whole32.grid, 1});
    c->strideB = c->strideA;

    int rc = MI355CG_OK;
    auto cleanup = [&]() { mi355cg_destroy(c); return rc; };
    if (hipStreamCreateWithFlags(&c->stream, hipStreamNonBlocking) != hipSuccess) { rc = fail(MI355CG_ERR_HIP, "hipStreamCreate failed"); return cleanup(); }
    if ((rc = upload_item_tables(c))) return cleanup();
    const long long L = c->storage_len;
    { const int m = env_int("MI355CG_XSTEPS", 4); c->xsteps = m == 2 ? 2 : ((m == 8 && dtype == MI355CG_F64) ? 8 : 4); }
    if (!part && dtype == MI355CG_F64 && !getenv("MI355CG_XSTEPS")) {
        const char* xf = getenv("MI355CG_XFOLD");
        const int want = (xf && *xf) ? atoi(xf) : -1;
        if (want == 16 || want == 32) c->xfold = want;
        else if (want < 0 && c->g.own_len >= (4LL << 20)) {
            size_t mem_free = 0, mem_total = 0;
            if (hipMemGetInfo(&mem_free, &mem_total) == hipSuccess)
                for (int R : {32, 16}) if (c->xfold == 0 && sizeof(double) * (size_t)L * (size_t)R <= mem_total / 4) c->xfold = R;
        }
        c->fold_grid = std::max(0, env_int("MI355CG_XFOLD_GRID", 0));
        c->fold_nt = env_int("MI355CG_XFOLD_NT", 1) != 0;
    }
    Buf<double>* vecs[] = {&c->x, &c->r, &c->p[0], &c->p[1], &c->ap, &c->b, &c->u, &c->p[2], &c->p[3], &c->p[4], &c->p[5], &c->p[6], &c->p[7]};
    for (int k = 0; k < 7 + (c->xsteps - 2); ++k) if ((rc = Buf<double>::device_zeroed(*vecs[k], L))) return cleanup();
    if (dtype == MI355CG_F32_MIXED) {
        Buf<float>* fv[] = {&c->xf, &c->rf, &c->pf[0], &c->pf[1], &c->apf, &c->pf[2], &c->pf[3], &c->pf[4], &c->pf[5], &c->pf[6], &c->pf[7]};
        for (int k = 0; k < 5 + (c->xsteps - 2); ++k) if ((rc = Buf<float>::device_zeroed(*fv[k], L, "fp32 vector allocation failed"))) return cleanup();
    }
    if ((rc = Buf<double>::device_zeroed(c->packed, std::max<long long>(c->pk_len, 1)))) return cleanup();
    if ((rc = create_state(c, "state allocation failed"))) return cleanup();
    c->rec_width = kRecHeader + 2 * c->g.Pu;
    if ((rc = Buf<double>::device_zeroed(c->sumsA, c->rec_width))) return cleanup();
    if ((rc = Buf<double>::device_zeroed(c->sumsB, c->rec_width))) return cleanup();
    if ((rc = Buf<int>::device_zeroed(c->qctr, 2 * kXcds * kQueueSubs * kQueuePitch, "queue counter allocation failed"))) return cleanup();
    if ((rc = Buf<int>::pinned(c->stop_h, 1, "stop word allocation failed"))) return cleanup();
    *c->stop_h = 0;
    if (hipDeviceSynchronize() != hipSuccess) { rc = fail(MI355CG_ERR_HIP, "hipDeviceSynchronize failed"); return cleanup(); }

    if (env_int("MI355CG_DEVICE_SETUP", 0)) {
        c->host_rhs_valid = false; c->host_u_valid = false;
        if ((rc = mi355cg_setup_on_device(c))) return cleanup();
    } else {
        c->rhs_h.resize(c->pk_len); c->u_h.resize(c->pk_len);
        grid_fill_box(gp, c->g.y_lo, c->g.y_hi, s_lo * kStripCols, s_hi == ns_all ? gp.n : s_hi * kStripCols, c->rhs_h.data(), c->u_h.data(), nullptr, nullptr);
        if ((rc = upload_packed<double>(c, c->rhs_h.data(), c->b))) return cleanup();
    }
    if (env_int("MI355CG_ONCHIP", 0) == 1 && !onchip_refusal(c)) c->solve_mode = MI355CG_SOLVE_ONCHIP;
    *out = c;
    return MI355CG_OK;
}

int mi355cg_create(int n, int m, double a, double b, double c_, double d, int dtype, int device, mi355cg_handle* out) {
    return create_impl(n, m, a, b, c_, d, dtype, device, 0, 0, 0, 0, false, out);
}
int mi355cg_create_slab(int n, int m, double a, double b, double c_, double d, int dtype, int device,
                        int y_lo, int y_hi, mi355cg_handle* out) {
    GridParams gp;
    if (!grid_params_init(&gp, n, m, a, b, c_, d)) return fail(MI355CG_ERR_INVALID, "grid %dx%d rejected: the L-shaped index map is only consistent for n == m, even, >= 6", n, m);
    return create_impl(n, m, a, b, c_, d, dtype, device, y_lo, y_hi, 0, strips_total(gp, 2), true, out);
}
int mi355cg_create_part(int n, int m, double a, double b, double c_, double d, int dtype, int device,
                        int y_lo, int y_hi, int x_lo, int x_hi, mi355cg_handle* out) {
    GridParams gp;
    if (!grid_params_init(&gp, n, m, a, b, c_, d)) return fail(MI355CG_ERR_INVALID, "grid %dx%d rejected: the L-shaped index map is only consistent for n == m, even, >= 6", n, m);
    const int ns_all = strips_total(gp, 2);
    if (x_lo % kStripCols != 0 || (x_hi % kStripCols != 0 && x_hi < gp.n))
        return fail(MI355CG_ERR_INVALID, "part columns [%d, %d): x-cuts must be multiples of %d", x_lo, x_hi, kStripCols);
    return create_impl(n, m, a, b, c_, d, dtype, device, y_lo, y_hi, x_lo / kStripCols, x_hi >= gp.n ? ns_all : x_hi / kStripCols, true, out);
}

int mi355cg_create_csr(long long nrows, const int* row_map, const int* entries, const double* values,
                       int device, mi355cg_handle* out) {
    if (!out) return fail(MI355CG_ERR_INVALID, "out is null");
    *out = nullptr;
    if (nrows <= 0 || !row_map || !entries || !values) return fail(MI355CG_ERR_INVALID, "bad CSR arguments");
    if (row_map[0] != 0) return fail(MI355CG_ERR_INVALID, "row_map[0] must be 0");
    const long long nnz = row_map[nrows];
    for (long long i = 0; i < nrows; ++i) if (row_map[i + 1] < row_map[i]) return fail(MI355CG_ERR_INVALID, "row_map is not monotone at row %lld", i);
    for (long long j = 0; j < nnz; ++j) if (entries[j] < 0 || entries[j] >= nrows) return fail(MI355CG_ERR_INVALID, "column index %d out of range at entry %lld", entries[j], j);
    int ndev = 0;
    if (hipGetDeviceCount(&ndev) != hipSuccess || ndev <= 0) return fail(MI355CG_ERR_HIP, "no HIP device available (libmi355cg has no CPU fallback)");
    if (device < 0 || device >= ndev) return fail(MI355CG_ERR_INVALID, "device %d out of range (0..%d)", device, ndev - 1);
    HIPCK(hipSetDevice(device));
    mi355cg_ctx* c = new mi355cg_ctx();
    c->device = device; c->dtype = MI355CG_F64; c->is_csr = true;
    c->csr_n = nrows; c->csr_nnz = nnz;
    c->gp.size = nrows; c->pk_begin = 0; c->pk_len = nrows; c->storage_len = nrows; c->pg.pk_len = nrows;
    c->g.own_begin = 0; c->g.own_len = nrows;
    const long long nblk = (nrows + kBlock - 1) / kBlock;
    c->grid_csr = (int)std::max<long long>(1, std::min<long long>(2048, nblk));
    c->grid_update = (int)std::max<long long>(1, std::min<long long>(512, nblk));
    c->strideA = c->grid_csr; c->strideB = c->grid_update; c->nB_own = c->grid_update;
    int rc = MI355CG_OK;
    auto cleanup = [&]() { mi355cg_destroy(c); return rc; };
    if (hipStreamCreateWithFlags(&c->stream, hipStreamNonBlocking) != hipSuccess) { rc = fail(MI355CG_ERR_HIP, "hipStreamCreate failed"); return cleanup(); }
    for (Buf<double>* v : {&c->x, &c->r, &c->p[0], &c->p[1], &c->ap, &c->b, &c->u}) if ((rc = Buf<double>::device_zeroed(*v, nrows))) return cleanup();
    if ((rc = create_state(c, "allocation failed"))) return cleanup();
    if ((rc = Buf<int>::device(c->csr_row_map, nrows + 1, "allocation failed")) || (rc = Buf<int>::device(c->csr_entries, std::max<long long>(nnz, 1), "allocation failed")) ||
        (rc = Buf<double>::device(c->csr_values, std::max<long long>(nnz, 1), "allocation failed"))) return cleanup();
    if (hipMemcpy(c->csr_row_map, row_map, sizeof(int) * (nrows + 1), hipMemcpyHostToDevice) != hipSuccess ||
        hipMemcpy(c->csr_entries, entries, sizeof(int) * nnz, hipMemcpyHostToDevice) != hipSuccess ||
        hipMemcpy(c->csr_values, values, sizeof(double) * nnz, hipMemcpyHostToDevice) != hipSuccess) {
        rc = fail(MI355CG_ERR_HIP, "CSR upload failed"); return cleanup();
    }
    if (hipDeviceSynchronize() != hipSuccess) { rc = fail(MI355CG_ERR_HIP, "hipDeviceSynchronize failed"); return cleanup(); }
// ... 51 lines not shown
int mi355cg_setup_on_device(mi355cg_handle c) {
    if (!c) return fail(MI355CG_ERR_INVALID, "null handle");
    if (c->is_csr) return fail(MI355CG_ERR_INVALID, "a CSR handle has no grid to set up");
    HIPCK(hipSetDevice(c->device));
    if (c->is_slab) HIPCK(hipDeviceSynchronize());
    SetupArgs s{};
    s.pg = c->pg; s.a = c->gp.a; s.c = c->gp.c; s.x_step = c->gp.x_step; s.y_step = c->gp.y_step; s.xk = c->gp.x_k; s.yk = c->gp.y_k;
    s.n = c->gp.n; s.m = c->gp.m;
    if (c->pk_len > 0) hipLaunchKernelGGL(k_setup, dim3(flat_grid(c->pk_len)), dim3(kBlock), 0, c->stream, s, c->b, c->u);
    HIPCK(hipGetLastError());
    HIPCK(hipStreamSynchronize(c->stream));
    c->have_u_dev = true; c->host_rhs_valid = false; c->host_u_valid = false;
    return MI355CG_OK;
}
int mi355cg_set_rhs(mi355cg_handle c, const double* b) {
    if (!c || !b) return fail(MI355CG_ERR_INVALID, "null argument");
    HIPCK(hipSetDevice(c->device));
    c->host_rhs_valid = true;
    c->rhs_h.resize(c->pk_len);
    std::memcpy(c->rhs_h.data(), b, sizeof(double) * c->pk_len);
    return upload_packed<double>(c, c->rhs_h.data(), c->b);
}

int mi355cg_apply_device(mi355cg_handle c, const double* x_dev, double* y_dev) {
    if (!c || !x_dev || !y_dev) return fail(MI355CG_ERR_INVALID, "null argument");
    if (c->is_slab) return fail(MI355CG_ERR_STATE, "this handle owns one part of a decomposed grid: use the mi355cg_team_* / mi355cg_dist_* entry points");
    HIPCK(hipSetDevice(c->device));
    if (c->is_csr) {
        launch_csr_spmv(c, x_dev, y_dev, nullptr, nullptr, nullptr);
        HIPCK(hipGetLastError());
        HIPCK(hipStreamSynchronize(c->stream));
        return MI355CG_OK;
    }
    if (int rc = ensure_scratch(c)) return rc;
    hipLaunchKernelGGL((k_unpack<double>), dim3(flat_grid(c->pk_len)), dim3(kBlock), 0, c->stream, c->pg, x_dev, c->scratch[0]);
    launch_apply<double, 2>(c, c->scratch[0], c->scratch[1], whole_part(c));
    hipLaunchKernelGGL((k_pack<double>), dim3(flat_grid(c->pk_len)), dim3(kBlock), 0, c->stream, c->pg, c->scratch[1], y_dev);
    HIPCK(hipGetLastError());
    HIPCK(hipStreamSynchronize(c->stream));
    return MI355CG_OK;
}

int mi355cg_apply(mi355cg_handle c, const double* x, double* y) {
    if (!c || !x || !y) return fail(MI355CG_ERR_INVALID, "null argument");
    if (c->is_slab) return fail(MI355CG_ERR_STATE, "this handle owns one part of a decomposed grid: use the mi355cg_team_* / mi355cg_dist_* entry points");
    HIPCK(hipSetDevice(c->device));
    if (int rc = ensure_scratch(c)) return rc;
    if (int rc = upload_packed<double>(c, x, c->scratch[0])) return rc;
    if (c->is_csr) launch_csr_spmv(c, c->scratch[0], c->scratch[1], nullptr, nullptr, nullptr);
    else launch_apply<double, 2>(c, c->scratch[0], c->scratch[1], whole_part(c));
    HIPCK(hipGetLastError());
    return download_packed<double>(c, c->scratch[1], y);
}

void mi355cg_default_params(mi355cg_params* p, int rule) {
    if (!p) return;
    std::memset(p, 0, sizeof *p);
    p->rule = rule;
    p->max_iterations = 10000;
    p->eps_precision = 1e-6; p->eps_residual = 1e-6; p->eps_exact_error = 1e-6;
    p->eps_rel = 1e-6;
    p->use_true_solution = 1;
    p->callback_every = rule == MI355CG_RULE_MSG_MAXNORM ? 100 : 1;
    p->diagnostics = 0;
    p->sync_every = 0;
    p->fixed_iterations = 0;
    p->inner_eps = 0.0;
}

static int launch_init_guess(mi355cg_ctx* c, bool has_u) {
    launch_apply<double, 2>(c, c->x, c->scratch[0], whole_part(c));
    GuessArgs<double> f{};
    f.begin = c->g.own_begin / 2; f.nvec = c->g.own_len / 2;
    f.b = c->b; f.ax = c->scratch[0]; f.x = c->x; f.r = c->r; f.p0 = c->p[0]; f.u = c->u;
    f.partB = c->partB; f.strideB = c->strideB; f.partG = c->guess_part; f.strideG = c->strideB; f.s_out = c->sB;
    if (has_u) hipLaunchKernelGGL((k_init_guess<double, 2, true>), dim3(c->whole.grid), dim3(kBlock), 0, c->stream, f);
    else hipLaunchKernelGGL((k_init_guess<double, 2, false>), dim3(c->whole.grid), dim3(kBlock), 0, c->stream, f);
    double* norms = c->guess_part + 2 * (size_t)c->strideB;
    hipLaunchKernelGGL(k_guess_state, dim3(1), dim3(kBlock), 0, c->stream, (const double*)c->partB, c->strideB, (const double*)c->guess_part, c->strideB,
                       c->whole.grid, c->sB, norms);
    HIPCK(hipMemcpyAsync(c->guess_norms_h, norms, sizeof(double) * 2, hipMemcpyDeviceToHost, c->stream));
    return MI355CG_OK;
}
static void launch_init_fresh(mi355cg_ctx* c, bool has_u) {
    FreshArgs<double> f{};
    f.begin = c->g.own_begin / 2; f.nvec = c->g.own_len / 2;
    f.b = c->b; f.x = c->x; f.r = c->r; f.p0 = c->p[0]; f.u = c->u;
    f.partB = c->partB; f.strideB = c->strideB; f.s_out = c->sB;
    if (has_u) hipLaunchKernelGGL((k_init_fresh<double, 2, true>), dim3(c->whole.grid), dim3(kBlock), 0, c->stream, f);
    else hipLaunchKernelGGL((k_init_fresh<double, 2, false>), dim3(c->whole.grid), dim3(kBlock), 0, c->stream, f);
}

static void launch_onchip_chunk(mi355cg_ctx* c, const IterCfg& cfg, const mi355cg_params* prm, int m) {
    OnchipArgs a{};
    a.g = c->g; a.pl = onchip_plan(c->gp.n);
    a.x = c->x; a.r = c->r; a.u = c->u;
    for (int k = 0; k < c->xsteps; ++k) a.p[k] = c->p[k];
    a.xsteps = c->xsteps;
    a.partB = c->partB; a.nB = c->nB_own; a.strideB = c->strideB;
    a.s = c->sB; a.hist = c->hist; a.rp = cfg.rp;
    a.has_u = cfg.has_u ? 1 : 0; a.u_always = cfg.rp.eps_exact_error > 0 ? 1 : 0; a.every = prm->callback_every;
    a.m = m; a.stop_req = c->stop_dev;
    const dim3 grid(1), block(a.pl.threads);
    const bool msg = cfg.rp.rule == MI355CG_RULE_MSG_MAXNORM;
#define MI355CG_OC(E) do { if (msg) hipLaunchKernelGGL((k_onchip<E, true>), grid, block, 0, c->stream, a); \
                           else hipLaunchKernelGGL((k_onchip<E, false>), grid, block, 0, c->stream, a); } while (0)
    switch (a.pl.elems) {
        case 1: MI355CG_OC(1); break;
        case 2: MI355CG_OC(2); break;
        case 4: MI355CG_OC(4); break;
        case 8: MI355CG_OC(8); break;
        case 16: MI355CG_OC(16); break;
        default: MI355CG_OC(kOnchipMaxElems); break;
    }
#undef MI355CG_OC
    c->nB_own = 1;
    ++c->onchip_launches;
}

int mi355cg_solve(mi355cg_handle c, const mi355cg_params* prm, mi355cg_iter_cb cb, void* user,
                  const volatile int* stop_flag, mi355cg_results* out) {
    if (!c || !prm) return fail(MI355CG_ERR_INVALID, "null argument");
    if (prm->rule != MI355CG_RULE_MSG_MAXNORM && prm->rule != MI355CG_RULE_REL_2NORM) return fail(MI355CG_ERR_INVALID, "unknown rule %d", prm->rule);
    if (c->is_slab) return fail(MI355CG_ERR_STATE, "this handle owns one part of a decomposed grid: use the mi355cg_team_* / mi355cg_dist_* entry points");
    HIPCK(hipSetDevice(c->device));
    const bool warm = c->guess_pending;
    c->guess_pending = false;
    c->onchip_launches = 0;
    if (c->is_csr) return solve_csr(c, prm, cb, user, stop_flag, out);
    if (c->dtype == MI355CG_F32_MIXED) return solve_mixed(c, prm, cb, user, stop_flag, out);
    if (c->mg) return solve_mg(c, prm, cb, user, stop_flag, out, warm);
    const bool msg = prm->rule == MI355CG_RULE_MSG_MAXNORM;
    IterCfg cfg0 = make_cfg(prm);
    const bool onchip = c->solve_mode == MI355CG_SOLVE_ONCHIP && cfg0.want_diag == 0;
    if (onchip) cfg0.x2 = false;
    cfg0.fold = cfg0.x2 && ensure_fold_ring(c);
    const IterCfg cfg = cfg0;
    const bool diag = cfg.want_diag != 0, fold = cfg.fold;
    c->nB_own = c->whole.grid;
    if (cfg.has_u) if (int rc = ensure_u_on_device(c)) return rc;
    if (diag || (warm && !(c->scratch[0] && c->scratch[1]))) if (int rc = ensure_scratch(c)) return rc;
    if (warm) if (int rc = ensure_guess_ws(c)) return rc;

    const auto t0 = std::chrono::steady_clock::now();
    c->events.reset(); c->ev_pairs[0].clear(); c->ev_pairs[1].clear();

    c->cur = 0; c->fcur = 0;
    if (c->qctr && c->dyn_rows > 0) HIPCK(hipMemsetAsync(c->qctr, 0, sizeof(int) * 2 * kXcds * kQueueSubs * kQueuePitch, c->stream));
    if (warm) { if (int rc = launch_init_guess(c, cfg.has_u)) return rc; }
    else launch_init_fresh(c, cfg.has_u);
    HIPCK(hipGetLastError());

    *c->stop_h = 0;
    c->stop_dev = nullptr;
    if (stop_flag) HIPCK(hipHostGetDevicePointer((void**)&c->stop_dev, c->stop_h, 0));
    auto wait_stream = [&]() -> int { return wait_stream_forwarding_stop(c, stop_flag); };
    bool polled = false;
    auto poll = [&]() -> int {
        launch_check(c, cfg, c->stream, own_partB(c));
        if (int rc = fetch_state(c, c->stream)) return rc;
        polled = true;
        return wait_stream();
    };
    *c->summary_h = CgState{};
    if (msg && (cb || warm)) {
        if (int rc = poll()) return rc;
        if (cb) cb(user, 0, DBL_MAX, c->summary_h->rmax, cfg.has_u ? c->summary_h->emax : DBL_MAX);
    }
    if (warm)
        if (const int reason = msg_stop_reason(prm, false, 0.0, c->summary_h->rmax, cfg.has_u, c->summary_h->emax)) {
            c->summary_h->done = 1; c->summary_h->converged = 1; c->summary_h->reason = reason;
        }
    if (int rc = loop_timer_begin(c, c->stream)) return rc;

    const int every = prm->callback_every;
    auto need_u = [&](int it) { return diag || cfg.rp.eps_exact_error > 0 || it == 1 || (every > 0 && it % every == 0); };
    const int sync_every = default_sync_every(prm, msg);
    int it_done = 0;
    bool interrupted = false;
    bool first_chunk = cb != nullptr || stop_flag != nullptr;
    if (std::memcmp(&c->graph_prm, prm, sizeof *prm) != 0 || c->graph_stop != (stop_flag != nullptr)) {
        clear_graphs(c); c->graph_prm = *prm; c->graph_stop = stop_flag != nullptr;
    }
    const bool graph_ok = !c->profiling && !diag &&
                          (c->use_graph == 1 || (c->use_graph < 0 && c->g.own_len < (4LL << 20) && prm->max_iterations >= 4 * sync_every));
    while (!c->summary_h->done) {
        if (stop_flag && *stop_flag) { interrupted = true; break; }
        const int m = chunk_len(prm, msg, sync_every, it_done, first_chunk);
        first_chunk = false;
        auto enqueue_chunk = [&]() -> int {
            for (int k = 0; k < m; ++k) {
                hipEvent_t e0 = nullptr;
                Buf<double> pp[kRing];
                if (fold) { pp[c->cur].borrow(c->fold_p[c->fcur]); pp[(c->cur + 1) % c->xsteps].borrow(c->fold_p[(c->fcur + 1) % c->xfold]); }
                const Buf<double>* ring = fold ? pp : c->p;
                prof_begin(c, &e0);
                launch_iteration_stencil<double, 2>(c, cfg, c->r, ring, whole_part(c), own_partB(c));
                c->cur = (c->cur + 1) % c->xsteps;
                if (fold) c->fcur = (c->fcur + 1) % c->xfold;
                prof_end(c, 0, e0);
                prof_begin(c, &e0);
                IterCfg ucfg = cfg;
                ucfg.has_u = cfg.has_u && need_u(it_done + k + 1);
                launch_iteration_update<double, 2>(c, ucfg, c->x, c->r, ring, c->u, whole_part(c), own_partA(c));
                if (fold && c->fcur == 0) launch_fold_x(c, -1, c->stream);
                prof_end(c, 1, e0);
                if (diag) {
                    launch_apply<double, 2>(c, c->x, c->scratch[0], whole_part(c));
                    hipLaunchKernelGGL((k_resid2<double>), dim3(1024), dim3(kBlock), 0, c->stream, c->g.own_begin, c->g.own_len, c->b, c->scratch[0], c->partR);
                    hipLaunchKernelGGL(k_resid2_hist, dim3(1), dim3(kBlock), 0, c->stream, c->partR, 1024, c->sB, c->hist);
                }
            }
            return MI355CG_OK;
        };
        if (onchip) {
            launch_onchip_chunk(c, cfg, prm, m);
        } else if (graph_ok && m >= 8) {
            std::vector<char> flags(m);
            for (int k = 0; k < m; ++k) flags[k] = cfg.has_u && need_u(it_done + k + 1);
            mi355cg_ctx::ChunkGraph* hit = nullptr;
            const int key = fold ? c->fcur : c->cur;
            for (auto& g : c->graphs) if (g.m == m && g.cur == key && g.flags == flags) hit = &g;
            if (!hit) {
                hipGraph_t graph = nullptr; hipGraphExec_t exec = nullptr;
                const int cur0 = c->cur, fcur0 = c->fcur;
                HIPCK(hipStreamBeginCapture(c->stream, hipStreamCaptureModeThreadLocal));
                const int rc = enqueue_chunk();
                const hipError_t e1 = hipStreamEndCapture(c->stream, &graph);
                c->cur = cur0; c->fcur = fcur0;
                if (rc) return rc;
                HIPCK(e1);
                HIPCK(hipGraphInstantiate(&exec, graph, nullptr, nullptr, 0));
                HIPCK(hipGraphDestroy(graph));
                c->graphs.push_back({m, key, flags, exec});
                hit = &c->graphs.back();
            }
            HIPCK(hipGraphLaunch(hit->exec, c->stream));
            c->cur = (c->cur + m) % c->xsteps;
            if (fold) c->fcur = (c->fcur + m) % c->xfold;
        } else {
            if (int rc = enqueue_chunk()) return rc;
        }
        HIPCK(hipGetLastError());
        if (int rc = poll()) return rc;
        const int it_now = c->summary_h->it;
        replay_callbacks(cb, user, prm, *c->summary_h, c->hist_h, it_done, it_now, cfg.has_u, diag);
        it_done = it_now;
    }
    if (int rc = loop_timer_end(c, c->stream)) return rc;
    CgState fin = *c->summary_h;
    c->stop_dev = nullptr;
    if (fin.done && fin.reason == MI355CG_STOP_INTERRUPTED) interrupted = true;
    c->cur = fin.it % c->xsteps;
    if (cfg.x2) {
        if (fold) { c->fcur = fin.it % c->xfold; if (c->fcur != 0) launch_fold_x(c, fin.it, c->stream); }
        else launch_flush_x<double, 2>(c, c->whole, c->x, c->p, fin, c->stream);
        HIPCK(hipGetLastError());
        HIPCK(hipStreamSynchronize(c->stream));
    }
    if (cfg.has_u && fin.it > 0 && !need_u(fin.it)) {
        hipLaunchKernelGGL((k_err_maxnorm<double>), dim3(1024), dim3(kBlock), 0, c->stream, c->g.own_begin, c->g.own_len, c->x, c->u, c->partR);
        HIPCK(hipGetLastError());
        HIPCK(hipMemcpyAsync(c->partR_h, c->partR, sizeof(double) * 1024, hipMemcpyDeviceToHost, c->stream));
        HIPCK(hipStreamSynchronize(c->stream));
        double m = 0; for (int i = 0; i < 1024; ++i) m = std::max(m, c->partR_h[i]);
        fin.emax = m;
    }
    c->solved = true; c->x_is_guess = false;
    prof_collect(c);
#ifdef MI355CG_WAVE_TIMING
    if (const char* path = getenv("MI355CG_WAVE_TIMING_OUT")) {
        std::vector<unsigned long long> buf(2 * kWtStamps * kWtWaves);
        HIPCK(hipMemcpyFromSymbol(buf.data(), HIP_SYMBOL(g_wave_dbg), buf.size() * sizeof(unsigned long long)));
        if (FILE* f = fopen(path, "wb")) { fwrite(buf.data(), sizeof(unsigned long long), buf.size(), f); fclose(f); }
    }
#endif
    mi355cg_results res = make_results(fin, interrupted, cfg.has_u, warm && polled ? c->guess_norms_h[0] : fin.r0norm);
    res.solve_seconds = std::chrono::duration<double>(std::chrono::steady_clock::now() - t0).count();
    HIPCK(hipEventSynchronize(c->ev_loop[1]));
    res.loop_seconds = loop_timer_seconds(c);
    if (msg && cb) cb(user, res.iterations, res.final_precision, res.final_residual_norm, res.final_error_norm);
    if (out) *out = res;
    return MI355CG_OK;
}

int mi355cg_get_solution(mi355cg_handle c, double* x) {
    if (!c || !x) return fail(MI355CG_ERR_INVALID, "null argument");
    if (c->x_is_guess) return fail(MI355CG_ERR_STATE, "an initial guess was set after the last solve: x holds the guess, not a solution");
    if (!c->solved) return fail(MI355CG_ERR_STATE, "no solve has run on this handle");
    HIPCK(hipSetDevice(c->device));
    return download_packed<double>(c, c->x, x);
}
int mi355cg_get_recursive_residual(mi355cg_handle c, double* r) {
    if (!c || !r) return fail(MI355CG_ERR_INVALID, "null argument");
    if (c->x_is_guess) return fail(MI355CG_ERR_STATE, "an initial guess was set after the last solve: r is not the residual of x");
    if (!c->solved) return fail(MI355CG_ERR_STATE, "no solve has run on this handle");
    HIPCK(hipSetDevice(c->device));
    return download_packed<double>(c, c->r, r);
}
int mi355cg_get_true_residual(mi355cg_handle c, double* out) {
    if (!c || !out) return fail(MI355CG_ERR_INVALID, "null argument");
    if (c->is_slab) return fail(MI355CG_ERR_STATE, "this handle owns one part of a decomposed grid: use the mi355cg_team_* / mi355cg_dist_* entry points");
    if (c->x_is_guess) return fail(MI355CG_ERR_STATE, "an initial guess was set after the last solve: x holds the guess, not a solution");
    if (!c->solved) return fail(MI355CG_ERR_STATE, "no solve has run on this handle");
    HIPCK(hipSetDevice(c->device));
    if (int rc = ensure_scratch(c)) return rc;
    if (c->is_csr) launch_csr_spmv(c, c->x, c->scratch[0], nullptr, nullptr, nullptr);
    else launch_apply<double, 2>(c, c->x, c->scratch[0], whole_part(c));
    hipLaunchKernelGGL((k_sub<double>), dim3(flat_grid(c->g.own_len)), dim3(kBlock), 0, c->stream, c->g.own_begin, c->g.own_len, c->scratch[0], c->b, c->scratch[1]);
    HIPCK(hipGetLastError());
    return download_packed<double>(c, c->scratch[1], out);
}

static int guess_check(mi355cg_ctx* c) {
    if (!c) return fail(MI355CG_ERR_INVALID, "null handle");
    if (c->is_csr) return fail(MI355CG_ERR_INVALID, "an initial guess needs the grid operator's start (r0 = b - A x0): a CSR handle has none");
    if (c->is_slab) return fail(MI355CG_ERR_INVALID, "an initial guess is single-GPU only: this handle owns one part of a decomposed grid");
    if (c->dtype != MI355CG_F64) return fail(MI355CG_ERR_INVALID, "an initial guess is fp64 only: this handle was created with MI355CG_F32_MIXED");
    return MI355CG_OK;
}

int mi355cg_set_initial_guess(mi355cg_handle c, const double* x0) {
    if (int rc = guess_check(c)) return rc;
    if (!x0) { c->guess_pending = false; return MI355CG_OK; }
    HIPCK(hipSetDevice(c->device));
    c->x_is_guess = true;
    if (int rc = upload_packed<double>(c, x0, c->x)) return rc;
    c->guess_pending = true;
    return MI355CG_OK;
}

int mi355cg_set_initial_guess_device(mi355cg_handle c, const double* x0_dev) {
    if (int rc = guess_check(c)) return rc;
    if (!x0_dev) return fail(MI355CG_ERR_INVALID, "null argument");
    HIPCK(hipSetDevice(c->device));
    c->x_is_guess = true;
    hipLaunchKernelGGL((k_unpack<double>), dim3(flat_grid(c->pk_len)), dim3(kBlock), 0, c->stream, c->pg, x0_dev, c->x);
    HIPCK(hipGetLastError());
    HIPCK(hipStreamSynchronize(c->stream));
    c->guess_pending = true;
    return MI355CG_OK;
// ... 55 lines not shown
    if (!c || !x_dev) return fail(MI355CG_ERR_INVALID, "null argument");
    if (c->x_is_guess) return fail(MI355CG_ERR_STATE, "an initial guess was set after the last solve: x holds the guess, not a solution");
    if (!c->solved) return fail(MI355CG_ERR_STATE, "no solve has run on this handle");
    HIPCK(hipSetDevice(c->device));
    if (c->is_csr) {
        HIPCK(hipMemcpyAsync(x_dev, c->x, sizeof(double) * c->pk_len, hipMemcpyDeviceToDevice, c->stream));
    } else {
        if (c->is_slab) HIPCK(hipDeviceSynchronize());
        if (c->pk_len > 0) hipLaunchKernelGGL((k_pack<double>), dim3(flat_grid(c->pk_len)), dim3(kBlock), 0, c->stream, c->pg, (const double*)c->x, x_dev);
        HIPCK(hipGetLastError());
    }
    HIPCK(hipStreamSynchronize(c->stream));
    return MI355CG_OK;
}

static void launch_step_rhs(mi355cg_ctx* c, double sigma, double theta) {
    StepRhsArgs a{};
    a.g = c->g;
    a.A0 = c->gp.A; a.xk = c->gp.x_k; a.yk = c->gp.y_k;
    a.sigma = sigma; a.theta = theta; a.c1 = (1.0 - theta) / theta;
    a.u = c->x; a.rhs = c->b; a.out = c->step_b;
    a.tiles_per_row = (c->g.N + kStepTileCols) / kStepTileCols;
    a.tiles = (long long)(c->g.N - 1) * a.tiles_per_row;
    const int grid = (int)std::min<long long>(a.tiles, 1 << 20);
    if (theta < 1.0) hipLaunchKernelGGL((k_step_rhs<true>), dim3(grid), dim3(kBlock), 0, c->stream, a);
    else hipLaunchKernelGGL((k_step_rhs<false>), dim3(grid), dim3(kBlock), 0, c->stream, a);
}

int mi355cg_time_steps(mi355cg_handle c, const mi355cg_params* prm, double tau, double theta, int nsteps,
                       const volatile int* stop_flag, mi355cg_results* out, int* steps_done) {
    if (!c || !prm || !out || !steps_done) return fail(MI355CG_ERR_INVALID, "null argument");
    if (int rc = shift_check(c)) return rc;
    if (!std::isfinite(tau) || !(tau > 0.0)) return fail(MI355CG_ERR_INVALID, "time step %g rejected: tau must be finite and > 0", tau);
    if (!(theta > 0.0 && theta <= 1.0)) return fail(MI355CG_ERR_INVALID, "theta %g rejected: the scheme needs 0 < theta <= 1", theta);
    if (nsteps < 0) return fail(MI355CG_ERR_INVALID, "nsteps %d rejected: it must be >= 0", nsteps);
    if (prm->rule != MI355CG_RULE_MSG_MAXNORM && prm->rule != MI355CG_RULE_REL_2NORM) return fail(MI355CG_ERR_INVALID, "unknown rule %d", prm->rule);
    if (prm->diagnostics) return fail(MI355CG_ERR_INVALID, "the stepper has no callbacks: diagnostics must be 0");
    if (prm->use_true_solution) return fail(MI355CG_ERR_INVALID, "a step has no exact solution: use_true_solution must be 0");
    const double sigma = 1.0 / (theta * tau);
    if (!std::isfinite(sigma)) return fail(MI355CG_ERR_INVALID, "time step %g rejected: 1 / (theta tau) is not finite", tau);
    if (nsteps == 0) { *steps_done = 0; return MI355CG_OK; }
    if (!c->guess_pending) return fail(MI355CG_ERR_STATE, "no starting state: set it with mi355cg_set_initial_guess* or mi355cg_use_solution_as_initial_guess");
    *steps_done = 0;
    HIPCK(hipSetDevice(c->device));
    if (!c->step_b) {
        if (int rc = Buf<double>::device_zeroed(c->step_b, c->storage_len)) return rc;
        HIPCK(hipDeviceSynchronize());
    }
    if (int rc = mi355cg_set_shift(c, sigma)) return rc;
    for (int k = 0; k < nsteps; ++k) {
        if (k > 0) { c->x_is_guess = true; c->guess_pending = true; }
        launch_step_rhs(c, sigma, theta);
        HIPCK(hipGetLastError());
        std::swap(c->b, c->step_b);
        const int rc = mi355cg_solve(c, prm, nullptr, nullptr, stop_flag, &out[k]);
        std::swap(c->b, c->step_b);
        if (rc) return rc;
        if (!out[k].converged) break;
        ++*steps_done;
    }
    return MI355CG_OK;
}

int mi355cg_set_profiling(mi355cg_handle c, int enable) {
    if (!c) return fail(MI355CG_ERR_INVALID, "null handle");
    c->profiling = enable != 0;
    return MI355CG_OK;
}
int mi355cg_get_kernel_time(mi355cg_handle c, int kernel, double* avg_ms, long long* launches) {
    if (!c || kernel < 0 || kernel > 1) return fail(MI355CG_ERR_INVALID, "bad argument");
    if (avg_ms) *avg_ms = c->kernel_ms[kernel];
    if (launches) *launches = c->kernel_launches[kernel];
    return MI355CG_OK;
}
int mi355cg_get_layout(mi355cg_handle c, long long* padded_len, int* pitch_bottom, int* pitch_upper,
                       int* grid_stencil, int* grid_update, int* rows_per_item) {
    if (!c) return fail(MI355CG_ERR_INVALID, "null handle");
    if (padded_len) *padded_len = c->g.own_len;
    if (pitch_bottom) *pitch_bottom = c->g.Pb;
    if (pitch_upper) *pitch_upper = c->g.Pu;
    if (grid_stencil) *grid_stencil = c->whole.grid;
    if (grid_update) *grid_update = c->whole.grid;
    if (rows_per_item) *rows_per_item = c->whole.ty;
    return MI355CG_OK;
}

int mi355cg_get_xfold(mi355cg_handle c, int* depth, int* extra_buffers) {
    if (!c) return fail(MI355CG_ERR_INVALID, "null handle");
    if (depth) *depth = c->xfold;
    if (extra_buffers) *extra_buffers = c->fold_extra;
    return MI355CG_OK;
}

int mi355cg_set_solve_mode(mi355cg_handle c, int mode) {
    if (!c) return fail(MI355CG_ERR_INVALID, "null handle");
    if (mode != MI355CG_SOLVE_LAUNCHES && mode != MI355CG_SOLVE_ONCHIP)
        return fail(MI355CG_ERR_INVALID, "unknown solve mode %d (MI355CG_SOLVE_LAUNCHES = 0, MI355CG_SOLVE_ONCHIP = 1)", mode);
    if (mode == MI355CG_SOLVE_ONCHIP) if (const char* why = onchip_refusal(c)) return fail(MI355CG_ERR_INVALID, "%s", why);
    if (mode == c->solve_mode) return MI355CG_OK;
    HIPCK(hipSetDevice(c->device));
    HIPCK(hipStreamSynchronize(c->stream));
    clear_graphs(c);
    c->solve_mode = mode;
    return MI355CG_OK;
}
int mi355cg_get_solve_mode(mi355cg_handle c, int* mode, long long* onchip_launches_last_solve) {
    if (!c) return fail(MI355CG_ERR_INVALID, "null handle");
    if (mode) *mode = c->solve_mode;
    if (onchip_launches_last_solve) *onchip_launches_last_solve = c->onchip_launches;
    return MI355CG_OK;
}
int mi355cg_onchip_plan(int n, int* threads, int* lds_bytes, int* elems_per_thread) {
    if (!onchip_supported(n))
        return fail(MI355CG_ERR_INVALID, "grid %d rejected: the on-chip solve takes even n from 6 to %d", n, kOnchipMaxN);
    const OnchipPlan pl = onchip_plan(n);
    if (threads) *threads = pl.threads;
    if (lds_bytes) *lds_bytes = pl.lds_bytes;
    if (elems_per_thread) *elems_per_thread = pl.elems;
    return MI355CG_OK;
}

int mi355cg_mg_levels(int n, int* levels, int* coarsest_n) {
    std::vector<int> ns;
    if (int rc = mg_shape(MI355CG_PRECOND_MG, n, &ns)) return rc;
    if (levels) *levels = (int)ns.size();
    if (coarsest_n) *coarsest_n = ns.back();
    return MI355CG_OK;
}

int mi355cg_mg_hierarchy(int kind, int n, int max_levels, int* levels, int* level_n) {
    if (max_levels < 0 || (max_levels > 0 && !level_n)) return fail(MI355CG_ERR_INVALID, "level_n must hold max_levels >= 0 entries");
    std::vector<int> ns;
    if (int rc = mg_shape(kind, n, &ns)) return rc;
    if (levels) *levels = (int)ns.size();
    for (int l = 0; l < (int)ns.size() && l < max_levels; ++l) level_n[l] = ns[l];
    return MI355CG_OK;
}

int mi355cg_set_preconditioner(mi355cg_handle c, int kind) { return mi355cg_set_preconditioner_ex(c, kind, MI355CG_CYCLE_F64); }

int mi355cg_set_preconditioner_ex(mi355cg_handle c, int kind, int cycle) {
    if (!c) return fail(MI355CG_ERR_INVALID, "null handle");
    if (kind != MI355CG_PRECOND_NONE && kind != MI355CG_PRECOND_MG && kind != MI355CG_PRECOND_MG_ANY)
        return fail(MI355CG_ERR_INVALID, "unknown preconditioner kind %d (MI355CG_PRECOND_NONE = 0, MI355CG_PRECOND_MG = 1, "
                    "MI355CG_PRECOND_MG_ANY = 2)", kind);
    HIPCK(hipSetDevice(c->device));
    if (kind == MI355CG_PRECOND_NONE) {
        mg_batch_free(c);
        eig_free(c);
        if (c->mg) { HIPCK(hipStreamSynchronize(c->stream)); c->mg.reset(); }
        return MI355CG_OK;
    }
    if (c->is_csr) return fail(MI355CG_ERR_INVALID, "the multigrid preconditioner needs the grid operator: a CSR handle has no grid");
    if (c->is_slab) return fail(MI355CG_ERR_INVALID, "the multigrid preconditioner is single-GPU only: this handle owns one part of a decomposed grid");
    if (c->dtype != MI355CG_F64) return fail(MI355CG_ERR_INVALID, "the multigrid preconditioner is fp64 only: this handle was created with MI355CG_F32_MIXED");
    if (c->solve_mode == MI355CG_SOLVE_ONCHIP)
        return fail(MI355CG_ERR_INVALID, "this handle is in the on-chip solve mode, which runs plain CG: mi355cg_set_solve_mode(h, MI355CG_SOLVE_LAUNCHES) first");
    std::vector<int> ns;
    if (int rc = mg_shape(kind, c->gp.n, &ns)) return rc;
    if (cycle != MI355CG_CYCLE_F64 && cycle != MI355CG_CYCLE_F32)
        return fail(MI355CG_ERR_INVALID, "unknown V-cycle precision %d (MI355CG_CYCLE_F64 = 0, MI355CG_CYCLE_F32 = 1)", cycle);
    if (cycle == MI355CG_CYCLE_F32 && c->smoother != MI355CG_SMOOTHER_JACOBI)
        return fail(MI355CG_ERR_INVALID, "the fp32 V-cycle smooths with point Jacobi only: this handle has line smoother %d "
                    "(mi355cg_set_smoother(h, MI355CG_SMOOTHER_JACOBI) first)", c->smoother);
    mg_batch_free(c);
    eig_free(c);
// ... 647 lines not shown
```

iterative_solvers_amd/csrc/solve_loop.h:

```cpp
#pragma once
#include "../../include/mi355cg.h"
#include <algorithm>
#include <cfloat>
#include <cmath>

namespace mi355cg {

constexpr int kHist = 512;
constexpr int kRing = 8;

struct CgState {
    double alpha, beta;
    double rr;
    double rr_prev;
    double rz;
    double r0norm;
    double rnorm2;
    double rmax, dmax, emax, d2, e2;
    int it, done, reason, converged, first;
    int stop;
    double alpha_hist[kRing];
};
struct HistEntry { double dmax, rmax, emax, rnorm2, d2, e2, tr2; };

inline int default_sync_every(const mi355cg_params* prm, bool msg) {
    return std::min(prm->sync_every > 0 ? prm->sync_every : (msg ? 100 : 200), kHist);
}
inline int chunk_len(const mi355cg_params* prm, bool msg, int sync_every, int it_done, bool first_chunk) {
    const int every = prm->callback_every;
    int m = std::min(sync_every, prm->max_iterations - it_done);
    if (msg && every > 0) m = std::min(m, every - it_done % every);
    if (first_chunk) m = 1;
    return std::max(m, 1);
}

inline void replay_callbacks(mi355cg_iter_cb cb, void* user, const mi355cg_params* prm, const CgState& fin, const HistEntry* hist_h,
                             int it_done, int it_now, bool has_u, bool diag) {
    if (!cb || !(diag || prm->rule == MI355CG_RULE_MSG_MAXNORM)) return;
    const int every = prm->callback_every;
    for (int it = it_done + 1; it <= it_now; ++it) {
        const HistEntry& h = hist_h[it % kHist];
        if (diag) { cb(user, it - 1, std::sqrt(h.d2), std::sqrt(h.tr2), std::sqrt(h.e2)); continue; }
        const bool stopped_here = fin.done && fin.reason != MI355CG_STOP_ITERATIONS && fin.reason != MI355CG_STOP_INTERRUPTED && it == it_now;
        if ((it == 1 || (every > 0 && it % every == 0)) && !stopped_here) cb(user, it, h.dmax, h.rmax, has_u ? h.emax : DBL_MAX);
    }
}

inline int msg_stop_reason(const mi355cg_params* prm, bool have_precision, double dmax, double rmax, bool has_u, double emax) {
    if (prm->rule != MI355CG_RULE_MSG_MAXNORM || prm->fixed_iterations) return 0;
    if (have_precision && prm->eps_precision > 0 && dmax < prm->eps_precision) return MI355CG_STOP_PRECISION;
    if (prm->eps_residual > 0 && rmax < prm->eps_residual) return MI355CG_STOP_RESIDUAL;
    if (prm->eps_exact_error > 0 && has_u && emax < prm->eps_exact_error) return MI355CG_STOP_EXACT_ERROR;
    return 0;
}

inline mi355cg_results make_results(int it, bool interrupted, int converged, int reason, double dmax, double rmax, bool has_u, double emax,
                                    double r_norm2, double initial_r_norm2) {
    mi355cg_results res{};
    res.iterations = it;
    res.converged = interrupted ? 0 : converged;
    res.stop_reason = interrupted ? MI355CG_STOP_INTERRUPTED : reason;
    res.final_residual_norm = rmax;
    res.final_precision = it > 0 ? dmax : DBL_MAX;
    res.final_error_norm = has_u ? emax : DBL_MAX;
    res.r_norm2 = r_norm2; res.initial_r_norm2 = initial_r_norm2;
    return res;
}
inline mi355cg_results make_results(const CgState& fin, bool interrupted, bool has_u, double initial_r_norm2) {
    return make_results(fin.it, interrupted, fin.converged, fin.reason, fin.dmax, fin.rmax, has_u, fin.emax, fin.rnorm2, initial_r_norm2);
}
inline mi355cg_results make_mixed_results(int it, bool interrupted, bool converged, double rnorm, double bnorm, int outer) {
    mi355cg_results res{};
    res.iterations = it; res.converged = converged ? 1 : 0;
    res.stop_reason = interrupted ? MI355CG_STOP_INTERRUPTED : (converged ? MI355CG_STOP_RESIDUAL : MI355CG_STOP_ITERATIONS);
    res.final_residual_norm = res.final_precision = res.final_error_norm = DBL_MAX;
    res.r_norm2 = rnorm; res.initial_r_norm2 = bnorm;
    res.refine_outer = outer; res.refine_true_rel = bnorm > 0 ? rnorm / bnorm : 0.0;
    return res;
}

}
```

iterative_solvers_amd/solver.py:

```python
from __future__ import annotations

import ctypes as C
import enum
import sys
from dataclasses import dataclass, field
from typing import Callable, Optional

import numpy as np

from . import _capi

DBL_MAX = sys.float_info.max
BATCH_MAX = _capi.BATCH_MAX


class StopCriterion(enum.IntEnum):
    ITERATIONS = 0
    PRECISION = 1
    RESIDUAL = 2
    EXACT_ERROR = 3
    INTERRUPTED = 4


_STOP_TEXT = {
# ... 304 lines not shown
        return np.ascontiguousarray(v)

    def eigs(self, nev: int, block: int, tol: float, max_iterations: int, x, stop_flag: Optional[C.c_int] = None):
        nev, block = int(nev), int(block)
        on_device = not isinstance(x, np.ndarray)
        if on_device:
            if not (type(x).__module__.split(".")[0] == "torch" and hasattr(x, "data_ptr")):
                raise ValueError(f"a start block is a NumPy array or a CUDA torch tensor, not {type(x).__name__}")
            import torch
            if not x.is_cuda:
                raise ValueError("a torch start block must be in device memory (a CPU tensor: pass tensor.numpy())")
            if x.dtype != torch.float64:
                raise ValueError(f"start block has dtype {x.dtype}, expected torch.float64")
            if x.device.index != self._device:
                raise ValueError(f"start block is on {x.device}, the handle on device {self._device}")
        elif x.dtype != np.float64:
            raise ValueError(f"start block has dtype {x.dtype}, expected float64")
        if tuple(x.shape) != (block, self.size):
            raise ValueError(f"start block has shape {tuple(x.shape)}, expected ({block}, {self.size})")
        lam, res = np.zeros(max(block, 1)), np.zeros(max(block, 1))
        out = _capi.EigResults()
        sp = C.cast(C.pointer(stop_flag), C.c_void_p) if stop_flag is not None else None
        if on_device:
            v = x.contiguous().clone()
            torch.cuda.current_stream(x.device).synchronize()
            rc = self._lib.mi355cg_eigs_device(self._h, nev, block, float(tol), int(max_iterations), v.data_ptr(), lam.ctypes.data,
                                               res.ctypes.data, sp, C.byref(out))
        else:
            v = np.array(x, dtype=np.float64, order="C", copy=True)
            rc = self._lib.mi355cg_eigs(self._h, nev, block, float(tol), int(max_iterations), v.ctypes.data, lam.ctypes.data,
                                        res.ctypes.data, sp, C.byref(out))
        if rc == _capi.ERR_INVALID:
            raise ValueError(self._lib.mi355cg_last_error().decode())
        _capi.check(rc)
        return lam[:block], v, res[:block], out

    def eigs_release(self):
        _capi.check(self._lib.mi355cg_eigs_release(self._h))

    def block_gram(self, a, b, rows=None, cols=None):
        a = self._check_block(a, self.size, _capi.EIG_BASIS_MAX, "a")
        b = self._check_block(b, self.size, _capi.EIG_BASIS_MAX, "b")
        ia = None if rows is None else np.ascontiguousarray(rows, dtype=np.int32)
        ib = None if cols is None else np.ascontiguousarray(cols, dtype=np.int32)
        out = np.empty((a.shape[0] if ia is None else ia.size, b.shape[0] if ib is None else ib.size))
        rc = self._lib.mi355cg_block_gram_indexed(self._h, a.shape[0], a.ctypes.data, 0 if ia is None else ia.size,
                                                  None if ia is None else ia.ctypes.data, b.shape[0], b.ctypes.data,
                                                  0 if ib is None else ib.size, None if ib is None else ib.ctypes.data, out.ctypes.data)
        if rc == _capi.ERR_INVALID:
            raise ValueError(self._lib.mi355cg_last_error().decode())
        _capi.check(rc)
        return out

    def block_combine(self, s, coef):
        s = self._check_block(s, self.size, _capi.EIG_BASIS_MAX, "s")
        coef = np.ascontiguousarray(coef, dtype=np.float64)
        if coef.ndim != 2 or coef.shape[0] != s.shape[0] or not 1 <= coef.shape[1] <= _capi.EIG_BLOCK_MAX:
            raise ValueError(f"coef has shape {tuple(coef.shape)}, expected ({s.shape[0]}, 1 .. {_capi.EIG_BLOCK_MAX})")
        y = np.empty((coef.shape[1], self.size))
        rc = self._lib.mi355cg_block_combine(self._h, s.shape[0], s.ctypes.data, coef.shape[1], coef.ctypes.data, y.ctypes.data)
        if rc == _capi.ERR_INVALID:
            raise ValueError(self._lib.mi355cg_last_error().decode())
        _capi.check(rc)
        return y

    def setup_on_device(self):
        _capi.check(self._lib.mi355cg_setup_on_device(self._h))

    def set_profiling(self, on: bool):
        _capi.check(self._lib.mi355cg_set_profiling(self._h, 1 if on else 0))

    def kernel_time(self, kernel: int):
        ms, n = C.c_double(), C.c_longlong()
        _capi.check(self._lib.mi355cg_get_kernel_time(self._h, kernel, C.byref(ms), C.byref(n)))
        return ms.value, n.value

    def layout(self):
        L = C.c_longlong()
        v = [C.c_int() for _ in range(5)]
        _capi.check(self._lib.mi355cg_get_layout(self._h, C.byref(L), *[C.byref(i) for i in v]))
        fold, extra = C.c_int(), C.c_int()
        if hasattr(self._lib, "mi355cg_get_xfold"):
            _capi.check(self._lib.mi355cg_get_xfold(self._h, C.byref(fold), C.byref(extra)))
        return {"padded_len": L.value, "pitch_bottom": v[0].value, "pitch_upper": v[1].value,
                "grid_stencil": v[2].value, "grid_update": v[3].value, "rows_per_item": v[4].value,
                "x_fold": fold.value, "x_fold_buffers": extra.value}


def default_params(rule: int) -> _capi.Params:
    p = _capi.Params()
    _capi.load().mi355cg_default_params(C.byref(p), rule)
    return p


def mg_levels(n: int):
    L, nc = C.c_int(), C.c_int()
    lib = _capi.load()
    rc = lib.mi355cg_mg_levels(int(n), C.byref(L), C.byref(nc))
    if rc == _capi.ERR_INVALID:
        raise ValueError(lib.mi355cg_last_error().decode())
    _capi.check(rc)
    return L.value, nc.value


def mg_hierarchy(n: int, kind: int = _capi.PRECOND_MG_ANY):
    L = C.c_int()
    buf = (C.c_int * 64)()
    lib = _capi.load()
    rc = lib.mi355cg_mg_hierarchy(int(kind), int(n), len(buf), C.byref(L), buf)
    if rc == _capi.ERR_INVALID:
        raise ValueError(lib.mi355cg_last_error().decode())
    _capi.check(rc)
    return tuple(buf[:L.value])


def onchip_plan(n: int):
    t, lds, e = C.c_int(), C.c_int(), C.c_int()
    lib = _capi.load()
    rc = lib.mi355cg_onchip_plan(int(n), C.byref(t), C.byref(lds), C.byref(e))
    if rc == _capi.ERR_INVALID:
        raise ValueError(lib.mi355cg_last_error().decode())
    _capi.check(rc)
    return {"threads": t.value, "lds_bytes": lds.value, "elems_per_thread": e.value}


def rayleigh_ritz(g, h):
    g = np.ascontiguousarray(g, dtype=np.float64)
    h = np.ascontiguousarray(h, dtype=np.float64)
    if g.ndim != 2 or g.shape[0] != g.shape[1] or h.shape != g.shape:
        raise ValueError(f"G and H are square matrices of one size, not {tuple(g.shape)} and {tuple(h.shape)}")
    k = g.shape[0]
    theta, coef = np.empty(max(k, 1)), np.empty((max(k, 1), max(k, 1)))
    lib = _capi.load()
    rc = lib.mi355cg_rayleigh_ritz(k, g.ctypes.data, h.ctypes.data, theta.ctypes.data, coef.ctypes.data)
    if rc == _capi.ERR_INVALID:
        raise ValueError(lib.mi355cg_last_error().decode())
    _capi.check(rc)
    return theta, coef


class MatrixFreeSystem:

    def __init__(self, m, n, a, b, c, d, device: int = 0, dtype: int = _capi.F64):
        self.n, self.m = n, m
        self.domain = (a, b, c, d)
        self._handle = _Handle(n, m, a, b, c, d, dtype=dtype, device=device)

    def get_rhs(self) -> np.ndarray: return self._handle.rhs()
    def get_true_solution_vector(self) -> np.ndarray: return self._handle.true_solution()
    def size(self) -> int: return self._handle.size

    def apply(self, x, y=None) -> np.ndarray:
        out = self._handle.apply(x)
        if y is not None:
            y[...] = out
            return y
        return out

    def __mul__(self, x): return self.apply(x)

    def set_preconditioner(self, kind: int, cycle: int = _capi.CYCLE_F64):
        self._handle.set_preconditioner(kind, cycle)

    def preconditioner_info(self):
        return self._handle.preconditioner_info()

    def set_solve_mode(self, mode: int):
        self._handle.set_solve_mode(mode)

# ... 291 lines not shown
```

Measured before the change: 8445 iters/s.

## Fuse cold-start init into first CG iteration and overlap final x-fold flush

For cold REL_2NORM f64 solves with x-folding, the init kernel now only computes the norm of b without writing x, r and p. The first iteration reads r from b and p from a zeroed buffer, and the fold kernel starts from zero instead of reading x. The final poll also skips the history copy when no callbacks replay it, and the tail x-fold flush is queued together with the last poll, avoiding an extra sync. This removes a full-vector write pass and some host round trips, at the cost of an extra zeroed buffer and more graph keys and branches.

```diff
diff --git a/include/mi355cg.h b/include/mi355cg.h
--- a/include/mi355cg.h
+++ b/include/mi355cg.h
@@ -154,6 +154,7 @@
 int  mi355cg_get_layout(mi355cg_handle h, long long *padded_len, int *pitch_bottom, int *pitch_upper,
                         int *grid_stencil, int *grid_update, int *rows_per_item);
 int  mi355cg_get_xfold(mi355cg_handle h, int *depth, int *extra_buffers);
+int  mi355cg_get_cold_start(mi355cg_handle h, int *in_place);
 
 #define MI355CG_SOLVE_LAUNCHES 0
 #define MI355CG_SOLVE_ONCHIP   1
diff --git a/iterative_solvers_amd/_capi.py b/iterative_solvers_amd/_capi.py
--- a/iterative_solvers_amd/_capi.py
+++ b/iterative_solvers_amd/_capi.py
@@ -28,7 +28,7 @@
     "mi355cg_team_set_profiling", "mi355cg_team_phase_times", "mi355cg_team_describe", "mi355cg_setup_on_device", "mi355cg_team_setup_on_device", "mi355cg_debug_plan",
     "mi355cg_team_set_dtype", "mi355cg_set_preconditioner", "mi355cg_apply_preconditioner", "mi355cg_mg_levels",
     "mi355cg_mg_hierarchy", "mi355cg_set_preconditioner_ex", "mi355cg_preconditioner_info",
-    "mi355cg_solve_batch", "mi355cg_solve_batch_device", "mi355cg_batch_release", "mi355cg_get_xfold",
+    "mi355cg_solve_batch", "mi355cg_solve_batch_device", "mi355cg_batch_release", "mi355cg_get_xfold", "mi355cg_get_cold_start",
     "mi355cg_set_initial_guess", "mi355cg_set_initial_guess_device", "mi355cg_use_solution_as_initial_guess",
     "mi355cg_solve_batch_from", "mi355cg_solve_batch_device_from",
     "mi355cg_set_shift", "mi355cg_get_shift", "mi355cg_time_steps", "mi355cg_get_solution_device",
@@ -213,6 +213,8 @@
         L.mi355cg_solve_many_info.argtypes = [H, C.c_int, IP, IP, LLP]
     if hasattr(L, "mi355cg_get_xfold"):
         L.mi355cg_get_xfold.argtypes = [H, IP, IP]
+    if hasattr(L, "mi355cg_get_cold_start"):
+        L.mi355cg_get_cold_start.argtypes = [H, IP]
     _lib = L
     return L
 
diff --git a/iterative_solvers_amd/csrc/cg_kernels.h b/iterative_solvers_amd/csrc/cg_kernels.h
--- a/iterative_solvers_amd/csrc/cg_kernels.h
+++ b/iterative_solvers_amd/csrc/cg_kernels.h
@@ -871,7 +871,7 @@
     double* partB; int strideB;
     CgState* s_out;
 };
-template <typename T, int VEC, bool HAS_U>
+template <typename T, int VEC, bool HAS_U, bool STORE = true>
 __global__ __launch_bounds__(kBlock) void k_init_fresh(const FreshArgs<T> a) {
     typedef typename VecOf<T, VEC>::type vec_t;
     __shared__ double lds[2 * kWaves];
@@ -887,7 +887,26 @@
 #pragma unroll
     for (int j = 0; j < VEC; ++j) zero[j] = (T)0;
     const long long end = a.begin + a.nvec;
-    for (long long i = a.begin + (long long)blockIdx.x * kBlock + threadIdx.x; i < end; i += stride) {
+    long long i = a.begin + (long long)blockIdx.x * kBlock + threadIdx.x;
+    if constexpr (!STORE) {
+        static_assert(STORE || !HAS_U, "the norm pass without stores serves REL_2NORM solves without u");
+        constexpr int kInFlight = 8;
+        for (; i + (kInFlight - 1) * stride < end; i += kInFlight * stride) {
+            vec_t bv[kInFlight];
+#pragma unroll
+            for (int k = 0; k < kInFlight; ++k) bv[k] = B[i + k * stride];
+#pragma unroll
+            for (int k = 0; k < kInFlight; ++k) {
+#pragma unroll
+                for (int j = 0; j < VEC; ++j) {
+                    const double rd = (double)bv[k][j];
+                    dd_acc_prod(s_rr, rd, rd);
+                    s_rmax = fmax(s_rmax, fabs(rd));
+                }
+            }
+        }
+    }
+    for (; i < end; i += stride) {
         const vec_t bv = B[i];
         vec_t uv; if (HAS_U) uv = Uu[i];
 #pragma unroll
@@ -901,7 +920,7 @@
                 dd_acc_prod(s_e2, ee, ee);
             }
         }
-        X[i] = zero; R[i] = bv; P[i] = zero;
+        if (STORE) { X[i] = zero; R[i] = bv; P[i] = zero; }
     }
     const dd t_rr = block_reduce_dd(s_rr, lds);
     const double t_rmax = block_reduce<true>(s_rmax, lds);
@@ -1002,10 +1021,12 @@
     QueueSpec dq;
     double* fold_alpha;
     int fold_mask;
+    const T* r_in;
 };
 
-template <typename T, int VEC, int XM, bool HAS_U, int DEPTH, bool DESC, bool TEAM, bool QUEUE>
+template <typename T, int VEC, int XM, bool HAS_U, int DEPTH, bool DESC, bool TEAM, bool QUEUE, bool RIN = false>
 __global__ __launch_bounds__(kBlock) void k_update_st(const UpdateStArgs<T> a) {
+    static_assert(!RIN || (XM == 0 && !TEAM), "RIN: the first iteration of a cold in-place solve, lean XM = 0 launches only");
     static_assert(DEPTH >= 1 && DEPTH <= 3, "see k_stencil");
     typedef typename VecOf<T, VEC>::type vec_t;
     __shared__ double lds[2 * kWaves];
@@ -1043,7 +1064,7 @@
         if (QUEUE && dq) dq_ticket = queue_take(dq, lane);
         F = item_addr<T, VEC, DESC>(g, u, lane);
         rs_p = make_rsrc(a.p + F.base_el);
-        rs_r = make_rsrc(a.r + F.base_el);
+        rs_r = make_rsrc((RIN ? a.r_in : a.r) + F.base_el);
         rs_x = make_rsrc(XM != 0 ? a.x + F.base_el : a.p + F.base_el);
 #pragma unroll
         for (int i = 0; i < NP; ++i) rs_pp[i] = make_rsrc(a.pprev[i] + F.base_el);
@@ -1311,6 +1332,8 @@
     const CgState* s;
     int mask;
     int flush_it;
+    const CgState* summary;
+    int x_cold;
 };
 template <int NS, bool NT>
 __device__ inline void fold_block(VecOf<double, 2>::type& xv, const FoldTable* tab, int k0, int mask, long long i) {
@@ -1330,17 +1353,17 @@
 template <bool NT>
 __global__ __launch_bounds__(kBlock) void k_fold_x(const FoldArgs a) {
     typedef VecOf<double, 2>::type vec_t;
-    const int it = a.flush_it >= 0 ? a.flush_it : scalar_load(&a.s->it);
-    int n = it & a.mask;
-    if (a.flush_it < 0) {
-        if (scalar_load(&a.s->done) || n != 0 || it == 0) return;
-        n = a.mask + 1;
-    }
+    const bool in_loop = a.flush_it == -1;
+    const int it = a.flush_it >= 0 ? a.flush_it : scalar_load(in_loop ? &a.s->it : &a.summary->it);
+    const FoldWindow w = fold_window(it, a.mask, in_loop, in_loop && scalar_load(&a.s->done) != 0);
+    const int n = w.n;
     if (n == 0) return;
+    const bool from_zero = a.x_cold && w.from_zero;
     vec_t* __restrict__ X = reinterpret_cast<vec_t*>(a.x);
     const long long stride = (long long)gridDim.x * kBlock, end = a.begin + a.nvec;
     for (long long i = a.begin + (long long)blockIdx.x * kBlock + threadIdx.x; i < end; i += stride) {
-        vec_t xv = X[i];
+        vec_t xv = {0.0, 0.0};
+        if (!from_zero) xv = X[i];
         int k = it - n + 1;
         for (; k + 8 <= it + 1; k += 8) fold_block<8, NT>(xv, a.tab, k, a.mask, i);
         if (k + 4 <= it + 1) { fold_block<4, NT>(xv, a.tab, k, a.mask, i); k += 4; }
diff --git a/iterative_solvers_amd/csrc/mi355cg.hip b/iterative_solvers_amd/csrc/mi355cg.hip
--- a/iterative_solvers_amd/csrc/mi355cg.hip
+++ b/iterative_solvers_amd/csrc/mi355cg.hip
@@ -216,6 +216,9 @@
     int fcur = 0;
     int fold_grid = 0;
     bool fold_nt = true;
+    Buf<double> fold_zero;
+    bool cold_pass = false;
+    bool cold_in_place = false;
 
     struct ChunkGraph { int m, cur; std::vector<char> flags; hipGraphExec_t exec; };
     std::vector<ChunkGraph> graphs;
@@ -428,7 +431,8 @@
 }
 
 template <typename T, int VEC>
-void launch_iteration_update(mi355cg_ctx* c, const IterCfg& cfg, T* x, T* r, const Buf<T> p[kRing], const T* u, const Where& w, const PartSrc& pa, const FlagSpec* fl = nullptr) {
+void launch_iteration_update(mi355cg_ctx* c, const IterCfg& cfg, T* x, T* r, const Buf<T> p[kRing], const T* u, const Where& w, const PartSrc& pa, const FlagSpec* fl = nullptr,
+                             const T* r_in = nullptr) {
     if (w.plan->wl.nitems == 0) return;
     UpdateStArgs<T> a{};
     a.g = kernel_geom<T, VEC>(c); a.tab = item_tab(*w.plan);
@@ -448,12 +452,22 @@
                                         else if (VEC == 2 && queue) hipLaunchKernelGGL((k_update_st<T, VEC, XM, HASU, D, true, false, VEC == 2>), grid, block, 0, w.stream, a); \
                                         else hipLaunchKernelGGL((k_update_st<T, VEC, XM, HASU, D, true, false, false>), grid, block, 0, w.stream, a); } while (0)
 #define MI355CG_UST(XM, HASU) do { if (d3) MI355CG_UST_D(XM, HASU, 3); else MI355CG_UST_D(XM, HASU, 2); } while (0)
-    if (cfg.x2) {
+    if (r_in) {}
+    else if (cfg.x2) {
         if (c->cur != 0 || cfg.fold) MI355CG_UST(0, false); else if (c->xsteps == 8) MI355CG_UST(8, false); else if (c->xsteps == 4) MI355CG_UST(4, false); else MI355CG_UST(2, false);
     }
     else if constexpr (VEC == 2) { if (cfg.has_u) MI355CG_UST(1, true); else MI355CG_UST(1, false); }
 #undef MI355CG_UST
 #undef MI355CG_UST_D
+    if (r_in) {
+        if constexpr (VEC == 2) {
+            a.r_in = r_in;
+            if (queue) { if (d3) hipLaunchKernelGGL((k_update_st<T, VEC, 0, false, 3, true, false, true, true>), grid, block, 0, w.stream, a);
+                         else hipLaunchKernelGGL((k_update_st<T, VEC, 0, false, 2, true, false, true, true>), grid, block, 0, w.stream, a); }
+            else { if (d3) hipLaunchKernelGGL((k_update_st<T, VEC, 0, false, 3, true, false, false, true>), grid, block, 0, w.stream, a);
+                   else hipLaunchKernelGGL((k_update_st<T, VEC, 0, false, 2, true, false, false, true>), grid, block, 0, w.stream, a); }
+        }
+    }
 }
 
 template <typename T, int VEC>
@@ -485,6 +499,7 @@
     FoldArgs a{};
     a.begin = c->g.own_begin / 2; a.nvec = c->g.own_len / 2;
     a.x = c->x; a.tab = c->fold_tab; a.s = c->sB; a.mask = c->xfold - 1; a.flush_it = flush_it;
+    a.summary = c->summary; a.x_cold = c->cold_in_place ? 1 : 0;
     const long long one_shot = (a.nvec + kBlock - 1) / kBlock;
     const int grid = (int)std::max<long long>(1, c->fold_grid > 0 ? std::min<long long>(c->fold_grid, one_shot) : one_shot);
     if (c->fold_nt) hipLaunchKernelGGL((k_fold_x<true>), dim3(grid), dim3(kBlock), 0, stream, a);
@@ -493,6 +508,7 @@
 void free_fold_ring(mi355cg_ctx* c) {
     for (int k = c->xsteps; k < kFoldMax; ++k) { c->fold_own[k].reset(); c->fold_p[k] = nullptr; }
     c->fold_tab.reset();
+    c->fold_zero.reset();
     c->fold_extra = 0;
 }
 bool ensure_fold_ring(mi355cg_ctx* c) {
@@ -507,6 +523,7 @@
     }
     FoldTable t{};
     for (int k = 0; k < c->xfold; ++k) t.p[k] = c->fold_p[k];
+    ok = ok && (c->cold_pass || (Buf<double>::device(c->fold_zero, c->storage_len) == MI355CG_OK && hipMemsetAsync(c->fold_zero, 0, bytes, c->stream) == hipSuccess));
     ok = ok && Buf<FoldTable>::device(c->fold_tab, 1) == MI355CG_OK &&
          hipMemcpyAsync(c->fold_tab, &t, sizeof t, hipMemcpyHostToDevice, c->stream) == hipSuccess && hipStreamSynchronize(c->stream) == hipSuccess;
     if (!ok) {
@@ -639,9 +656,9 @@
     c->events.reset();
 }
 
-int fetch_state(mi355cg_ctx* c, hipStream_t st) {
+int fetch_state(mi355cg_ctx* c, hipStream_t st, bool with_hist = true) {
     HIPCK(hipMemcpyAsync(c->summary_h, c->summary, sizeof(CgState), hipMemcpyDeviceToHost, st));
-    HIPCK(hipMemcpyAsync(c->hist_h, c->hist, sizeof(HistEntry) * kHist, hipMemcpyDeviceToHost, st));
+    if (with_hist) HIPCK(hipMemcpyAsync(c->hist_h, c->hist, sizeof(HistEntry) * kHist, hipMemcpyDeviceToHost, st));
     return MI355CG_OK;
 }
 int wait_stream_forwarding_stop(mi355cg_ctx* c, const volatile int* stop_flag) {
@@ -1868,6 +1885,8 @@
         c->fold_grid = std::max(0, env_int("MI355CG_XFOLD_GRID", 0));
         c->fold_nt = env_int("MI355CG_XFOLD_NT", 1) != 0;
     }
+    c->cold_pass = env_int("MI355CG_COLD_PASS", 0) == 1;
+    c->cold_in_place = c->xfold != 0 && !c->cold_pass;
     Buf<double>* vecs[] = {&c->x, &c->r, &c->p[0], &c->p[1], &c->ap, &c->b, &c->u, &c->p[2], &c->p[3], &c->p[4], &c->p[5], &c->p[6], &c->p[7]};
     for (int k = 0; k < 7 + (c->xsteps - 2); ++k) if ((rc = Buf<double>::device_zeroed(*vecs[k], L))) return cleanup();
     if (dtype == MI355CG_F32_MIXED) {
@@ -2085,13 +2104,14 @@
     HIPCK(hipMemcpyAsync(c->guess_norms_h, norms, sizeof(double) * 2, hipMemcpyDeviceToHost, c->stream));
     return MI355CG_OK;
 }
-static void launch_init_fresh(mi355cg_ctx* c, bool has_u) {
+static void launch_init_fresh(mi355cg_ctx* c, bool has_u, bool store = true) {
     FreshArgs<double> f{};
     f.begin = c->g.own_begin / 2; f.nvec = c->g.own_len / 2;
     f.b = c->b; f.x = c->x; f.r = c->r; f.p0 = c->p[0]; f.u = c->u;
     f.partB = c->partB; f.strideB = c->strideB; f.s_out = c->sB;
-    if (has_u) hipLaunchKernelGGL((k_init_fresh<double, 2, true>), dim3(c->whole.grid), dim3(kBlock), 0, c->stream, f);
-    else hipLaunchKernelGGL((k_init_fresh<double, 2, false>), dim3(c->whole.grid), dim3(kBlock), 0, c->stream, f);
+    if (store && has_u) hipLaunchKernelGGL((k_init_fresh<double, 2, true>), dim3(c->whole.grid), dim3(kBlock), 0, c->stream, f);
+    else if (store) hipLaunchKernelGGL((k_init_fresh<double, 2, false>), dim3(c->whole.grid), dim3(kBlock), 0, c->stream, f);
+    else hipLaunchKernelGGL((k_init_fresh<double, 2, false, false>), dim3(c->whole.grid), dim3(kBlock), 0, c->stream, f);
 }
 
 static void launch_onchip_chunk(mi355cg_ctx* c, const IterCfg& cfg, const mi355cg_params* prm, int m) {
@@ -2130,6 +2150,7 @@
     const bool warm = c->guess_pending;
     c->guess_pending = false;
     c->onchip_launches = 0;
+    c->cold_in_place = false;
     if (c->is_csr) return solve_csr(c, prm, cb, user, stop_flag, out);
     if (c->dtype == MI355CG_F32_MIXED) return solve_mixed(c, prm, cb, user, stop_flag, out);
     if (c->mg) return solve_mg(c, prm, cb, user, stop_flag, out, warm);
@@ -2140,6 +2161,12 @@
     cfg0.fold = cfg0.x2 && ensure_fold_ring(c);
     const IterCfg cfg = cfg0;
     const bool diag = cfg.want_diag != 0, fold = cfg.fold;
+    ColdStartIn cs{};
+    cs.warm = warm; cs.f64_single = c->dtype == MI355CG_F64 && !onchip; cs.rule = prm->rule;
+    cs.diagnostics = prm->diagnostics != 0; cs.use_true_solution = prm->use_true_solution != 0;
+    cs.fold = fold && c->fold_zero.get() != nullptr; cs.callback = cb != nullptr; cs.force_pass = c->cold_pass;
+    const bool cold = cold_start_in_place(cs);
+    c->cold_in_place = cold;
     c->nB_own = c->whole.grid;
     if (cfg.has_u) if (int rc = ensure_u_on_device(c)) return rc;
     if (diag || (warm && !(c->scratch[0] && c->scratch[1]))) if (int rc = ensure_scratch(c)) return rc;
@@ -2151,7 +2178,7 @@
     c->cur = 0; c->fcur = 0;
     if (c->qctr && c->dyn_rows > 0) HIPCK(hipMemsetAsync(c->qctr, 0, sizeof(int) * 2 * kXcds * kQueueSubs * kQueuePitch, c->stream));
     if (warm) { if (int rc = launch_init_guess(c, cfg.has_u)) return rc; }
-    else launch_init_fresh(c, cfg.has_u);
+    else launch_init_fresh(c, cfg.has_u, !cold);
     HIPCK(hipGetLastError());
 
     *c->stop_h = 0;
@@ -2159,10 +2186,21 @@
     if (stop_flag) HIPCK(hipHostGetDevicePointer((void**)&c->stop_dev, c->stop_h, 0));
     auto wait_stream = [&]() -> int { return wait_stream_forwarding_stop(c, stop_flag); };
     bool polled = false;
+    const bool replays = cb != nullptr && (diag || msg);
     auto poll = [&]() -> int {
         launch_check(c, cfg, c->stream, own_partB(c));
-        if (int rc = fetch_state(c, c->stream)) return rc;
+        if (int rc = fetch_state(c, c->stream, replays)) return rc;
         polled = true;
+        return wait_stream();
+    };
+    bool tail_queued = false;
+    auto poll_and_flush = [&]() -> int {
+        launch_check(c, cfg, c->stream, own_partB(c));
+        if (int rc = fetch_state(c, c->stream, replays)) return rc;
+        if (int rc = loop_timer_end(c, c->stream)) return rc;
+        launch_fold_x(c, -2, c->stream);
+        HIPCK(hipGetLastError());
+        polled = true; tail_queued = true;
         return wait_stream();
     };
     *c->summary_h = CgState{};
@@ -2194,18 +2232,19 @@
         auto enqueue_chunk = [&]() -> int {
             for (int k = 0; k < m; ++k) {
                 hipEvent_t e0 = nullptr;
+                const bool in_place = cold && it_done + k == 0;
                 Buf<double> pp[kRing];
-                if (fold) { pp[c->cur].borrow(c->fold_p[c->fcur]); pp[(c->cur + 1) % c->xsteps].borrow(c->fold_p[(c->fcur + 1) % c->xfold]); }
+                if (fold) { pp[c->cur].borrow(in_place ? c->fold_zero.get() : c->fold_p[c->fcur]); pp[(c->cur + 1) % c->xsteps].borrow(c->fold_p[(c->fcur + 1) % c->xfold]); }
                 const Buf<double>* ring = fold ? pp : c->p;
                 prof_begin(c, &e0);
-                launch_iteration_stencil<double, 2>(c, cfg, c->r, ring, whole_part(c), own_partB(c));
+                launch_iteration_stencil<double, 2>(c, cfg, in_place ? c->b.get() : c->r.get(), ring, whole_part(c), own_partB(c));
                 c->cur = (c->cur + 1) % c->xsteps;
                 if (fold) c->fcur = (c->fcur + 1) % c->xfold;
                 prof_end(c, 0, e0);
                 prof_begin(c, &e0);
                 IterCfg ucfg = cfg;
                 ucfg.has_u = cfg.has_u && need_u(it_done + k + 1);
-                launch_iteration_update<double, 2>(c, ucfg, c->x, c->r, ring, c->u, whole_part(c), own_partA(c));
+                launch_iteration_update<double, 2>(c, ucfg, c->x, c->r, ring, c->u, whole_part(c), own_partA(c), nullptr, in_place ? c->b.get() : nullptr);
                 if (fold && c->fcur == 0) launch_fold_x(c, -1, c->stream);
                 prof_end(c, 1, e0);
                 if (diag) {
@@ -2222,7 +2261,7 @@
             std::vector<char> flags(m);
             for (int k = 0; k < m; ++k) flags[k] = cfg.has_u && need_u(it_done + k + 1);
             mi355cg_ctx::ChunkGraph* hit = nullptr;
-            const int key = fold ? c->fcur : c->cur;
+            const int key = (fold ? c->fcur : c->cur) | (cold ? 1 << 16 : 0) | (cold && it_done == 0 ? 1 << 17 : 0);
             for (auto& g : c->graphs) if (g.m == m && g.cur == key && g.flags == flags) hit = &g;
             if (!hit) {
                 hipGraph_t graph = nullptr; hipGraphExec_t exec = nullptr;
@@ -2245,21 +2284,27 @@
             if (int rc = enqueue_chunk()) return rc;
         }
         HIPCK(hipGetLastError());
-        if (int rc = poll()) return rc;
+        if (fold && chunk_reaches_cap(prm, it_done, m)) { if (int rc = poll_and_flush()) return rc; }
+        else if (int rc = poll()) return rc;
         const int it_now = c->summary_h->it;
         replay_callbacks(cb, user, prm, *c->summary_h, c->hist_h, it_done, it_now, cfg.has_u, diag);
         it_done = it_now;
-    }
-    if (int rc = loop_timer_end(c, c->stream)) return rc;
+        if (tail_queued) break;
+    }
+    if (!tail_queued) if (int rc = loop_timer_end(c, c->stream)) return rc;
     CgState fin = *c->summary_h;
     c->stop_dev = nullptr;
     if (fin.done && fin.reason == MI355CG_STOP_INTERRUPTED) interrupted = true;
     c->cur = fin.it % c->xsteps;
     if (cfg.x2) {
-        if (fold) { c->fcur = fin.it % c->xfold; if (c->fcur != 0) launch_fold_x(c, fin.it, c->stream); }
+        if (fold) { c->fcur = fin.it % c->xfold; if (c->fcur != 0 && !tail_queued) launch_fold_x(c, fin.it, c->stream); }
         else launch_flush_x<double, 2>(c, c->whole, c->x, c->p, fin, c->stream);
+        if (cold && fin.it == 0) {
+            HIPCK(hipMemsetAsync(c->x + c->g.own_begin, 0, sizeof(double) * (size_t)c->g.own_len, c->stream));
+            HIPCK(hipMemcpyAsync(c->r + c->g.own_begin, c->b + c->g.own_begin, sizeof(double) * (size_t)c->g.own_len, hipMemcpyDeviceToDevice, c->stream));
+        }
         HIPCK(hipGetLastError());
-        HIPCK(hipStreamSynchronize(c->stream));
+        if (!tail_queued || (cold && fin.it == 0)) HIPCK(hipStreamSynchronize(c->stream));
     }
     if (cfg.has_u && fin.it > 0 && !need_u(fin.it)) {
         hipLaunchKernelGGL((k_err_maxnorm<double>), dim3(1024), dim3(kBlock), 0, c->stream, c->g.own_begin, c->g.own_len, c->x, c->u, c->partR);
@@ -2481,6 +2526,12 @@
     if (grid_stencil) *grid_stencil = c->whole.grid;
     if (grid_update) *grid_update = c->whole.grid;
     if (rows_per_item) *rows_per_item = c->whole.ty;
+    return MI355CG_OK;
+}
+
+int mi355cg_get_cold_start(mi355cg_handle c, int* in_place) {
+    if (!c) return fail(MI355CG_ERR_INVALID, "null handle");
+    if (in_place) *in_place = c->cold_in_place ? 1 : 0;
     return MI355CG_OK;
 }
 
diff --git a/iterative_solvers_amd/csrc/solve_loop.h b/iterative_solvers_amd/csrc/solve_loop.h
--- a/iterative_solvers_amd/csrc/solve_loop.h
+++ b/iterative_solvers_amd/csrc/solve_loop.h
@@ -32,6 +32,33 @@
     if (msg && every > 0) m = std::min(m, every - it_done % every);
     if (first_chunk) m = 1;
     return std::max(m, 1);
+}
+
+struct ColdStartIn {
+    bool warm;
+    bool f64_single;
+    int rule;
+    bool diagnostics, use_true_solution;
+    bool fold;
+    bool callback;
+    bool force_pass;
+};
+inline bool cold_start_in_place(const ColdStartIn& s) {
+    return !s.warm && s.f64_single && s.rule == MI355CG_RULE_REL_2NORM && !s.diagnostics && !s.use_true_solution && s.fold && !s.callback &&
+           !s.force_pass;
+}
+inline bool chunk_reaches_cap(const mi355cg_params* prm, int it_done, int m) { return it_done + m >= prm->max_iterations; }
+
+#ifdef __HIP__
+#define MI355CG_FOLD_HD __attribute__((host)) __attribute__((device))
+#else
+#define MI355CG_FOLD_HD
+#endif
+struct FoldWindow { int n; bool from_zero; };
+MI355CG_FOLD_HD inline FoldWindow fold_window(int it, int mask, bool in_loop, bool done) {
+    int n = it & mask;
+    if (in_loop) n = (done || n != 0 || it == 0) ? 0 : mask + 1;
+    return FoldWindow{n, n > 0 && it - n == 0};
 }
 
 inline void replay_callbacks(mi355cg_iter_cb cb, void* user, const mi355cg_params* prm, const CgState& fin, const HistEntry* hist_h,
diff --git a/iterative_solvers_amd/solver.py b/iterative_solvers_amd/solver.py
--- a/iterative_solvers_amd/solver.py
+++ b/iterative_solvers_amd/solver.py
@@ -410,9 +410,12 @@
         fold, extra = C.c_int(), C.c_int()
         if hasattr(self._lib, "mi355cg_get_xfold"):
             _capi.check(self._lib.mi355cg_get_xfold(self._h, C.byref(fold), C.byref(extra)))
+        in_place = C.c_int()
+        if hasattr(self._lib, "mi355cg_get_cold_start"):
+            _capi.check(self._lib.mi355cg_get_cold_start(self._h, C.byref(in_place)))
         return {"padded_len": L.value, "pitch_bottom": v[0].value, "pitch_upper": v[1].value,
                 "grid_stencil": v[2].value, "grid_update": v[3].value, "rows_per_item": v[4].value,
-                "x_fold": fold.value, "x_fold_buffers": extra.value}
+                "x_fold": fold.value, "x_fold_buffers": extra.value, "cold_start": "in_place" if in_place.value else "pass"}
 
 
 def default_params(rule: int) -> _capi.Params:
```

New measurement: 8452 iters/s (median of 3 runs). No clear change (+0.1%).
